# Deeptanshu-sankhwar/horizonml

Hardware: AMD Instinct MI355X
Metric: images/sec (higher is better)
Workload: dtype bf16; 1 GPU; model=resnet18_cifar10, global_batch=64, image=3x32x32, parallelism=dp1, optimizer=adam, exec=graph, comm=none

## Files before the change

### horizonml_amd/ops/csrc/bind.cpp

```cpp
#include <torch/extension.h>
#include <c10/hip/HIPStream.h>
#include <c10/hip/HIPCachingAllocator.h>

#include <memory>
#include <vector>

#include "launch.h"

namespace {

using torch::Tensor;

hipStream_t cur_stream() { return c10::hip::getCurrentHIPStream().stream(); }

bool g_deterministic = false;
void set_deterministic(bool on) {
  g_deterministic = on;
  set_kernels_deterministic(on ? 1 : 0);
}
bool deterministic_enabled() { return g_deterministic; }

void set_bn_owner(bool on) { set_kernels_bn_owner(on ? 1 : 0); }
bool bn_owner_enabled() { return kernels_bn_owner() != 0; }
std::vector<int64_t> bn_owner_launches() {
  long f = 0, b = 0;
  bn_owner_launch_counts(&f, &b);
  return {(int64_t)f, (int64_t)b};
}

bool g_dgrad_krsc = env_long("HZ_DGRAD_KRSC", 1) != 0;
void set_dgrad_krsc(bool on) { g_dgrad_krsc = on; }
bool dgrad_krsc_enabled() { return g_dgrad_krsc; }

bool g_wgrad_tr = env_long("HZ_WGRAD_TR", 1) != 0;
void set_wgrad_tr(bool on) { g_wgrad_tr = on; }
bool wgrad_tr_enabled() { return g_wgrad_tr; }

struct PendingWgrad {
  torch::Tensor x, dconv, dw;
  ConvP p;
};

bool g_wgrad_defer = false;
std::vector<PendingWgrad> g_pending;
torch::Tensor g_wgrad_ws;

void set_wgrad_defer(bool on) { g_wgrad_defer = on; }
bool wgrad_defer_enabled() { return g_wgrad_defer; }
int64_t wgrad_pending() { return (int64_t)g_pending.size(); }

static inline int cdiv_i(long a, long b) { return (int)((a + b - 1) / b); }

void flush_one_group(int lo, int hi);

void flush_wgrad() {
  if (g_pending.empty()) return;
  const int total = (int)g_pending.size();
  int lo = 0;
  while (lo < total) {
    std::vector<const void*> seen;
    int hi = lo;
    for (; hi < total; hi++) {
      const void* ptr = g_pending[hi].dw.data_ptr();
      bool dup = false;
      for (const void* q : seen)
        if (q == ptr) { dup = true; break; }
      if (dup) break;
      seen.push_back(ptr);
    }
    flush_one_group(lo, hi);
    lo = hi;
  }
  g_pending.clear();
}

void flush_wgrad_range(torch::Tensor flat, int64_t lo_elem, int64_t hi_elem) {
  if (g_pending.empty()) return;
  const char* base = (const char*)flat.data_ptr();
  const char* plo = base + lo_elem * flat.element_size();
  const char* phi = base + hi_elem * flat.element_size();
  std::vector<PendingWgrad> take, keep;
  for (auto& p : g_pending) {
    const char* q = (const char*)p.dw.data_ptr();
    if (q >= plo && q < phi)
      take.push_back(std::move(p));
    else
      keep.push_back(std::move(p));
  }
  g_pending = std::move(take);
  flush_wgrad();
  g_pending = std::move(keep);
}

void flush_one_group(int group_lo, int group_hi) {
  auto st = cur_stream();
  const int n = group_hi - group_lo;
  const PendingWgrad* pend = g_pending.data() + group_lo;
  std::vector<int> msplit(n), mchunk(n);
  std::vector<long> ws_off(n, 0);
  long ws_total = 0;
  for (int i = 0; i < n; i++) {
    const ConvP& p = pend[i].p;
    static const int mc_small = (int)env_long("HZ_WG_MCHUNK", 512);
    const int mc_base = p.M >= 32768 ? 2048 : mc_small;
    int ms = std::max(1, cdiv_i(p.M, mc_base));
    int mc = cdiv_i(cdiv_i(p.M, ms), 32) * 32;
    ms = cdiv_i(p.M, mc);
    msplit[i] = ms;
    mchunk[i] = mc;
    if (ms > 1) {
      ws_off[i] = ws_total;
      ws_total += (long)ms * p.K * p.Kd;
    }
  }
  if (ws_total > 0 &&
      (!g_wgrad_ws.defined() || g_wgrad_ws.numel() < ws_total))
    g_wgrad_ws = at::empty({ws_total},
                           pend[0].x.options().dtype(torch::kFloat32));
  float* ws_base = ws_total > 0 ? g_wgrad_ws.data_ptr<float>() : nullptr;

  auto tk3_of = [](const ConvP& p) {
    static const int kd_min = (int)env_long("HZ_WG_TK3_KD", 256);
    static const int m_min = (int)env_long("HZ_WG_TK3_M", 5000);
    return (p.Kd >= kd_min && p.M >= m_min) ? 128 : 64;
  };
  auto tko_of = [](const ConvP& p) {
    static const int k_min = (int)env_long("HZ_WG_TKO_K", 128);
    return p.K >= k_min ? 128 : 64;
  };
  for (int cls = 0; cls < 4; cls++) {
    const int tk3 = (cls & 1) ? 128 : 64;
    const int tko = (cls & 2) ? 128 : 64;
    std::vector<int> idx;
    for (int i = 0; i < n; i++)
      if (tk3_of(pend[i].p) == tk3 && tko_of(pend[i].p) == tko)
        idx.push_back(i);
    for (size_t lo = 0; lo < idx.size(); lo += WG_MAX_TASKS) {
      WgradBatchArgs a{};
      a.n = (int)std::min((size_t)WG_MAX_TASKS, idx.size() - lo);
      int blocks = 0;
      for (int j = 0; j < a.n; j++) {
        const int i = idx[lo + j];
        const PendingWgrad& pw = pend[i];
        WgradTask& t = a.t[j];
        t.X = pw.x.data_ptr();
        t.Dz = pw.dconv.data_ptr();
        t.out = msplit[i] > 1 ? ws_base + ws_off[i]
                              : pw.dw.data_ptr<float>();
        t.p = pw.p;
        t.mg = make_magic(pw.p, 1);
        t.Ntot = pw.p.K;
        t.mchunk = mchunk[i];
        t.msplit = msplit[i];
        t.tx = cdiv_i(pw.p.Kd, tk3);
        t.ty = cdiv_i(pw.p.K, tko);
        t.base = blocks;
        t.vec = (pw.p.C % 8) == 0;
        blocks += t.tx * t.ty * t.msplit;
      }
      launch_wgrad_batched_t(&a, blocks, tk3, tko, (int)g_wgrad_tr, st);
    }
  }

  WredBatchArgs r{};
  r.n = 0;
  int rblocks = 0;
  auto flush_red = [&]() {
    if (r.n > 0) launch_wgrad_reduce_batched(&r, rblocks, st);
    r.n = 0;
    rblocks = 0;
  };
  for (int i = 0; i < n; i++) {
    if (msplit[i] <= 1) continue;
    if (r.n == WG_MAX_TASKS) flush_red();
    WredTask& t = r.t[r.n++];
    t.ws = ws_base + ws_off[i];
    t.dW = pend[i].dw.data_ptr<float>();
    t.n = (long)pend[i].p.K * pend[i].p.Kd;
    t.msplit = msplit[i];
    t.base = rblocks;
    rblocks += cdiv_i(t.n, 1024);
  }
  flush_red();
}

void check_cl(const Tensor& t, const char* name) {
  TORCH_CHECK(t.is_cuda(), name, " must be on GPU");
  TORCH_CHECK(t.scalar_type() == torch::kBFloat16, name, " must be bf16");
  TORCH_CHECK(t.dim() == 4, name, " must be 4-D");
  bool cl = t.is_contiguous(at::MemoryFormat::ChannelsLast);
  bool hw1 = t.size(2) == 1 && t.size(3) == 1 && t.is_contiguous();
  TORCH_CHECK(cl || hw1, name, " must be channels_last contiguous");
}

void check_f32(const Tensor& t, const char* name) {
  TORCH_CHECK(t.is_cuda() && t.scalar_type() == torch::kFloat32 &&
                  t.is_contiguous(),
              name, " must be contiguous f32 on GPU");
}

template <class T>
T* opt_ptr(const c10::optional<Tensor>& t) {
  return t.has_value() ? t->data_ptr<T>() : nullptr;
}
void* opt_ptr(const c10::optional<Tensor>& t) {
  return t.has_value() ? t->data_ptr() : nullptr;
}

void check_probe(const c10::optional<Tensor>& prev,
                 const c10::optional<Tensor>& sumsq,
                 const c10::optional<Tensor>& out) {
  TORCH_CHECK(prev.has_value() == sumsq.has_value()
                  && prev.has_value() == out.has_value(),
              "probe tensors must be passed together");
}

Tensor empty_cl_bf16(int64_t n, int64_t c, int64_t h, int64_t w,
                     const Tensor& like) {
  return at::empty({n, c, h, w},
                   like.options().dtype(torch::kBFloat16),
                   at::MemoryFormat::ChannelsLast);
}

ConvP make_convp(const Tensor& x, int K, int R, int S, int stride, int pad) {
  ConvP p{};
  p.Nb = (int)x.size(0);
  p.C = (int)x.size(1);
  p.H = (int)x.size(2);
  p.W = (int)x.size(3);
  p.K = K;
  p.R = R;
  p.S = S;
  p.str = stride;
  p.pad = pad;
  p.Ho = (p.H + 2 * pad - R) / stride + 1;
  p.Wo = (p.W + 2 * pad - S) / stride + 1;
  p.M = p.Nb * p.Ho * p.Wo;
  p.Kd = R * S * p.C;
  return p;
}

std::vector<Tensor> conv_bn_act_fwd(
    Tensor x, Tensor w, Tensor gamma, Tensor beta, Tensor running_mean,
    Tensor running_var, int64_t stride, int64_t pad, double momentum,
    double eps, bool training, int64_t act,
    c10::optional<Tensor> residual, c10::optional<Tensor> stats_buf) {
  check_cl(x, "x");
  TORCH_CHECK(w.is_cuda() && w.scalar_type() == torch::kBFloat16 &&
                  w.is_contiguous() && w.dim() == 4,
              "w must be contiguous bf16 KRSC");
  check_f32(gamma, "gamma");
  check_f32(beta, "beta");
  int K = (int)w.size(0), R = (int)w.size(1), S = (int)w.size(2);
  TORCH_CHECK(w.size(3) == x.size(1), "w in-channels mismatch");
  ConvP p = make_convp(x, K, R, S, (int)stride, (int)pad);

  Tensor convout = empty_cl_bf16(p.Nb, K, p.Ho, p.Wo, x);
  Tensor y = empty_cl_bf16(p.Nb, K, p.Ho, p.Wo, x);
  auto fopt = x.options().dtype(torch::kFloat32);
  Tensor stats, smean, sinvstd;
  float* stats_ptr = nullptr;
  if (training) {
    smean = at::empty({K}, fopt);
    sinvstd = at::empty({K}, fopt);
  } else {
    smean = at::empty({0}, fopt);
    sinvstd = at::empty({0}, fopt);
  }
  const void* res_ptr = nullptr;
  if (residual.has_value()) {
    check_cl(*residual, "residual");
    res_ptr = residual->data_ptr();
  }
  auto st = cur_stream();
  int splitk = conv_fwd_splitk(p);
  const int own = (training && splitk > 1)
                      ? bn_owner_fwd_pick((long)p.M, K, 0) : 0;
  if (training && !own) {
    stats = stats_buf.has_value() ? *stats_buf : at::zeros({2L * K}, fopt);
    stats_ptr = stats.data_ptr<float>();
  }
  if (splitk > 1) {
    int kchunk = ((p.Kd + splitk - 1) / splitk + 31) / 32 * 32;
    splitk = (p.Kd + kchunk - 1) / kchunk;
    Tensor ws = at::empty({(long)splitk * p.M * K}, fopt);
    launch_conv_fwd_splitk(x.data_ptr(), w.data_ptr(), ws.data_ptr<float>(),
                           p, splitk, st);
    if (own) {
      launch_bn_fwd_owner(ws.data_ptr<float>(), res_ptr, y.data_ptr(),
                          convout.data_ptr(), gamma.data_ptr<float>(),
                          beta.data_ptr<float>(),
                          running_mean.data_ptr<float>(),
                          running_var.data_ptr<float>(),
                          smean.data_ptr<float>(), sinvstd.data_ptr<float>(),
                          (long)p.M, K, (float)momentum, (float)eps,
                          (int)act, splitk, own, st);
      return {y, convout, smean, sinvstd};
    }
    if (training)
      launch_stats_reduce(ws.data_ptr<float>(), stats_ptr, (long)p.M, K,
                          splitk, st);
    launch_bn_apply_f32(ws.data_ptr<float>(), res_ptr, y.data_ptr(),
                        convout.data_ptr(), stats_ptr,
                        gamma.data_ptr<float>(), beta.data_ptr<float>(),
                        running_mean.data_ptr<float>(),
                        running_var.data_ptr<float>(),
                        training ? smean.data_ptr<float>() : nullptr,
                        training ? sinvstd.data_ptr<float>() : nullptr,
                        (long)p.M, K, (float)momentum, (float)eps,
                        training ? 1 : 0, (int)act, splitk, st);
  } else {
    launch_conv_fwd(x.data_ptr(), w.data_ptr(), convout.data_ptr(),
                    g_deterministic ? nullptr : stats_ptr, p, st);
    if (g_deterministic && training)
      launch_stats_bf16_det(convout.data_ptr(), stats_ptr, (long)p.M, K,
                            st);
    launch_bn_apply(convout.data_ptr(), res_ptr, y.data_ptr(), stats_ptr,
                    gamma.data_ptr<float>(), beta.data_ptr<float>(),
                    running_mean.data_ptr<float>(),
                    running_var.data_ptr<float>(),
                    training ? smean.data_ptr<float>() : nullptr,
                    training ? sinvstd.data_ptr<float>() : nullptr,
                    (long)p.M, K, (float)momentum, (float)eps,
                    training ? 1 : 0, (int)act, st);
  }
  return {y, convout, smean, sinvstd};
}

Tensor dgrad_dx(const Tensor& dconv, const Tensor& w,
                const c10::optional<Tensor>& w_rsck, const ConvP& p,
                const c10::optional<Tensor>& dx_accum,
                const c10::optional<std::vector<Tensor>>& fuse_up,
                int up_mask_mode, hipStream_t st) {
  const bool krsc =
      !w_rsck.has_value() || w_rsck->data_ptr() == w.data_ptr();
  const Tensor& wt = krsc ? w : *w_rsck;
  TORCH_CHECK(wt.is_contiguous() && wt.scalar_type() == torch::kBFloat16,
              krsc ? "w must be contiguous bf16"
                   : "w_rsck must be contiguous bf16");
  TORCH_CHECK(wt.numel() == (int64_t)p.K * p.R * p.S * p.C,
              "dgrad weight has ", wt.numel(), " elements, expected K*R*S*C");
  auto fopt = dconv.options().dtype(torch::kFloat32);
  const int layout = krsc ? DGRAD_W_KRSC : DGRAD_W_RSCK;
  int accum = dx_accum.has_value() ? 1 : 0;
  Tensor dx = accum ? *dx_accum : empty_cl_bf16(p.Nb, p.C, p.H, p.W, dconv);
  ConvP pd = p;
  pd.M = p.Nb * p.H * p.W;
  pd.Kd = p.R * p.S * p.K;
  int splitk = conv_dgrad_splitk(p);
  const bool fuse = fuse_up.has_value();
  if (splitk > 1) {
    int kchunk = ((pd.Kd + splitk - 1) / splitk + 31) / 32 * 32;
    splitk = (pd.Kd + kchunk - 1) / kchunk;
    Tensor wsd = at::empty({(long)splitk * pd.M * p.C}, fopt);
    launch_conv_dgrad(dconv.data_ptr(), wt.data_ptr(), nullptr,
                      wsd.data_ptr<float>(), splitk, pd, 0, layout, st);
    if (fuse) {
      auto& f = *fuse_up;
      launch_cast_bnact(wsd.data_ptr<float>(), dx.data_ptr(), (long)pd.M,
                        p.C, splitk, accum, f[0].data_ptr(),
                        f[1].defined() ? f[1].data_ptr() : f[0].data_ptr(),
                        f[2].data_ptr<float>(), f[3].data_ptr<float>(),
                        f[4].data_ptr<float>(), f[5].data_ptr<float>(),
                        f[6].data_ptr<float>(), f[7].data_ptr<float>(),
                        up_mask_mode, st);
    } else {
      launch_cast_f32_bf16(wsd.data_ptr<float>(), dx.data_ptr(),
                           (long)pd.M * p.C, splitk, accum, st);
    }
  } else {
    launch_conv_dgrad(dconv.data_ptr(), wt.data_ptr(), dx.data_ptr(), nullptr,
                      1, pd, accum, layout, st);
    if (fuse) {
      auto& f = *fuse_up;
      launch_bnact_bwd_reduce(dx.data_ptr(), f[1].defined()
                                  ? f[1].data_ptr() : f[0].data_ptr(),
                              f[0].data_ptr(), f[2].data_ptr<float>(),
                              f[3].data_ptr<float>(),
                              f[4].data_ptr<float>(),
                              f[5].data_ptr<float>(),
                              f[6].data_ptr<float>(),
                              f[7].data_ptr<float>(), (long)pd.M, p.C,
                              up_mask_mode, st);
    }
  }
  return dx;
}

Tensor conv_dgrad_only(Tensor dz, Tensor w, int64_t H, int64_t W,
                       int64_t stride, int64_t pad,
                       c10::optional<Tensor> w_rsck,
                       c10::optional<Tensor> dx_accum) {
  check_cl(dz, "dz");
  TORCH_CHECK(w.dim() == 4 && w.size(0) == dz.size(1),
              "w must be [K,R,S,C] with K = dz channels");
  ConvP p{};
  p.Nb = (int)dz.size(0);
  p.C = (int)w.size(3);
  p.H = (int)H;
  p.W = (int)W;
  p.K = (int)w.size(0);
  p.R = (int)w.size(1);
  p.S = (int)w.size(2);
  p.str = (int)stride;
  p.pad = (int)pad;
  p.Ho = (p.H + 2 * p.pad - p.R) / p.str + 1;
  p.Wo = (p.W + 2 * p.pad - p.S) / p.str + 1;
  p.M = p.Nb * p.Ho * p.Wo;
  p.Kd = p.R * p.S * p.C;
  TORCH_CHECK(dz.size(2) == p.Ho && dz.size(3) == p.Wo,
              "dz spatial size does not match H, W, stride, pad");
  if (dx_accum.has_value()) {
    check_cl(*dx_accum, "dx_accum");
    TORCH_CHECK(dx_accum->size(0) == p.Nb && dx_accum->size(1) == p.C &&
                    dx_accum->size(2) == p.H && dx_accum->size(3) == p.W,
                "dx_accum must be [Nb,C,H,W]");
  }
  return dgrad_dx(dz, w, w_rsck, p, dx_accum, c10::nullopt, 0, cur_stream());
}

std::vector<Tensor> conv_bn_act_bwd(
    Tensor dy, Tensor y, Tensor x, Tensor w, c10::optional<Tensor> w_rsck,
    Tensor convout,
    Tensor gamma, Tensor beta, Tensor save_mean, Tensor save_invstd,
    int64_t stride, int64_t pad, int64_t act, bool need_dx, bool has_res,
    c10::optional<Tensor> dw_out, c10::optional<Tensor> dgamma_out,
    c10::optional<Tensor> dbeta_out, c10::optional<Tensor> dx_accum,
    c10::optional<std::vector<Tensor>> fuse_up, int64_t up_mask_mode,
    bool sums_ready, c10::optional<Tensor> sum_dz_in,
    c10::optional<Tensor> sum_dzx_in) {
  check_cl(dy, "dy");
  check_cl(y, "y");
  check_cl(x, "x");
  check_cl(convout, "convout");
  int K = (int)w.size(0), R = (int)w.size(1), S = (int)w.size(2);
  ConvP p = make_convp(x, K, R, S, (int)stride, (int)pad);
  auto fopt = x.options().dtype(torch::kFloat32);
  auto st = cur_stream();

  bool direct = dw_out.has_value();
  int mask_mode = act == 1 ? (has_res ? 1 : 2)
                 : act == 2 ? (has_res ? 3 : 4) : 0;
  Tensor sum_dz, sum_dzx;
  const int own = sums_ready ? 0 : bn_owner_bwd_pick((long)p.M, K, 0);
  if (sums_ready) {
    sum_dz = direct ? *dbeta_out : *sum_dz_in;
    sum_dzx = direct ? *dgamma_out : *sum_dzx_in;
  } else {
    sum_dz = direct ? *dbeta_out : at::zeros({K}, fopt);
    sum_dzx = direct ? *dgamma_out : at::zeros({K}, fopt);
    if (!own)
      launch_bnact_bwd_reduce(dy.data_ptr(), y.data_ptr(),
                              convout.data_ptr(),
                              save_mean.data_ptr<float>(),
                              save_invstd.data_ptr<float>(),
                              gamma.data_ptr<float>(),
                              beta.data_ptr<float>(),
                              sum_dz.data_ptr<float>(),
                              sum_dzx.data_ptr<float>(),
                              (long)p.M, K, mask_mode, st);
  }

  Tensor dconv = empty_cl_bf16(p.Nb, K, p.Ho, p.Wo, x);
  Tensor dres;
  void* dres_ptr = nullptr;
  if (has_res) {
    dres = empty_cl_bf16(p.Nb, K, p.Ho, p.Wo, x);
    dres_ptr = dres.data_ptr();
  }
  if (own)
    launch_bn_bwd_owner(dy.data_ptr(), y.data_ptr(), convout.data_ptr(),
                        save_mean.data_ptr<float>(),
                        save_invstd.data_ptr<float>(),
                        gamma.data_ptr<float>(), beta.data_ptr<float>(),
                        sum_dz.data_ptr<float>(), sum_dzx.data_ptr<float>(),
                        dconv.data_ptr(), dres_ptr, (long)p.M, K, mask_mode,
                        own, st);
  else
    launch_bn_bwd_apply(dy.data_ptr(), y.data_ptr(), convout.data_ptr(),
                        save_mean.data_ptr<float>(),
                        save_invstd.data_ptr<float>(),
                        gamma.data_ptr<float>(), beta.data_ptr<float>(),
                        sum_dz.data_ptr<float>(), sum_dzx.data_ptr<float>(),
                        dconv.data_ptr(), dres_ptr, (long)p.M, K, mask_mode,
                        st);

  Tensor dw = direct ? *dw_out
                     : at::zeros({(int64_t)K, R, S, (int64_t)p.C}, fopt);
  if (direct && g_wgrad_defer) {
    g_pending.push_back({x, dconv, dw, p});
  } else {
    int msplit = wgrad_msplit(p);
    Tensor ws;
    float* ws_ptr = nullptr;
    if (msplit > 1) {
      ws = at::empty({(long)msplit * K * p.Kd}, fopt);
      ws_ptr = ws.data_ptr<float>();
    }
    launch_wgrad(x.data_ptr(), dconv.data_ptr(), dw.data_ptr<float>(), ws_ptr,
                 p, (int)g_wgrad_tr, st);
  }

  TORCH_CHECK(need_dx || !fuse_up.has_value(),
              "fuse_up requires need_dx (the fused reduce rides the dx "
              "production)");
  Tensor dx;
  if (need_dx)
    dx = dgrad_dx(dconv, w, w_rsck, p, dx_accum, fuse_up, (int)up_mask_mode,
                  st);
  return {dx, dw, sum_dzx, sum_dz, dres};
}

void check_dw_geometry(int R, int S, int64_t stride, int H, int W,
                       int64_t pad) {
  TORCH_CHECK(R >= 1 && S >= 1 && R * S <= 25,
              "depthwise filter must have R*S <= 25 taps, got ", R, "x", S);
  TORCH_CHECK(stride >= 1, "depthwise stride must be >= 1, got ", stride);
  TORCH_CHECK(pad >= 0, "depthwise pad must be >= 0, got ", pad);
  TORCH_CHECK(H + 2 * pad >= R && W + 2 * pad >= S,
              "depthwise output must be at least 1x1: input ", H, "x", W,
              ", pad ", pad, ", filter ", R, "x", S);
}

std::vector<Tensor> dw_conv_bn_fwd(
    Tensor x, Tensor w, Tensor gamma, Tensor beta, Tensor running_mean,
    Tensor running_var, int64_t stride, int64_t pad, double momentum,
    double eps, bool training, int64_t act, c10::optional<Tensor> residual) {
  check_cl(x, "x");
  TORCH_CHECK(w.is_cuda() && w.scalar_type() == torch::kBFloat16 &&
                  w.is_contiguous() && w.dim() == 3,
              "w must be contiguous bf16 [R,S,C]");
  int Nb = (int)x.size(0), C = (int)x.size(1), H = (int)x.size(2),
      W = (int)x.size(3);
  int R = (int)w.size(0), S = (int)w.size(1);
  TORCH_CHECK((int)w.size(2) == C, "depthwise channel mismatch");
  check_dw_geometry(R, S, stride, H, W, pad);
  int Ho = (H + 2 * (int)pad - R) / (int)stride + 1;
  int Wo = (W + 2 * (int)pad - S) / (int)stride + 1;
  long M = (long)Nb * Ho * Wo;
  auto fopt = x.options().dtype(torch::kFloat32);
  Tensor convout = empty_cl_bf16(Nb, C, Ho, Wo, x);
  Tensor y = empty_cl_bf16(Nb, C, Ho, Wo, x);
  Tensor stats, smean, sinvstd;
  float* stats_ptr = nullptr;
  if (training) {
    stats = at::zeros({2L * C}, fopt);
    smean = at::empty({C}, fopt);
    sinvstd = at::empty({C}, fopt);
    stats_ptr = stats.data_ptr<float>();
  } else {
    smean = at::empty({0}, fopt);
    sinvstd = at::empty({0}, fopt);
  }
  const void* res_ptr = nullptr;
  if (residual.has_value()) {
    check_cl(*residual, "residual");
    res_ptr = residual->data_ptr();
  }
  auto st = cur_stream();
  launch_dw_fwd(x.data_ptr(), w.data_ptr(), convout.data_ptr(),
                g_deterministic ? nullptr : stats_ptr, Nb, H, W, C, Ho, Wo,
                R, S, (int)stride, (int)pad, st);
  if (g_deterministic && training)
    launch_stats_bf16_det(convout.data_ptr(), stats_ptr, M, C, st);
  launch_bn_apply(convout.data_ptr(), res_ptr, y.data_ptr(), stats_ptr,
                  gamma.data_ptr<float>(), beta.data_ptr<float>(),
                  running_mean.data_ptr<float>(),
                  running_var.data_ptr<float>(),
                  training ? smean.data_ptr<float>() : nullptr,
                  training ? sinvstd.data_ptr<float>() : nullptr, M, C,
                  (float)momentum, (float)eps, training ? 1 : 0, (int)act,
                  st);
  return {y, convout, smean, sinvstd};
}

std::vector<Tensor> dw_conv_bn_bwd(
    Tensor dy, Tensor y, Tensor x, Tensor w, Tensor convout, Tensor gamma,
    Tensor beta, Tensor save_mean, Tensor save_invstd, int64_t stride,
    int64_t pad, int64_t act, bool need_dx, bool has_res) {
  check_cl(dy, "dy");
  check_cl(x, "x");
  int Nb = (int)x.size(0), C = (int)x.size(1), H = (int)x.size(2),
      W = (int)x.size(3);
  TORCH_CHECK(w.is_cuda() && w.scalar_type() == torch::kBFloat16 &&
                  w.is_contiguous() && w.dim() == 3 && w.size(2) == C,
              "w must be contiguous bf16 [R,S,C] with C = x channels");
  int R = (int)w.size(0), S = (int)w.size(1);
  check_dw_geometry(R, S, stride, H, W, pad);
  int Ho = (int)dy.size(2), Wo = (int)dy.size(3);
  TORCH_CHECK(dy.size(0) == Nb && dy.size(1) == C &&
                  Ho == (H + 2 * (int)pad - R) / (int)stride + 1 &&
                  Wo == (W + 2 * (int)pad - S) / (int)stride + 1,
              "dy shape does not match the depthwise output of x");
  long M = (long)Nb * Ho * Wo;
  auto fopt = x.options().dtype(torch::kFloat32);
  auto st = cur_stream();
  int mask_mode = act == 1 ? (has_res ? 1 : 2)
                 : act == 2 ? (has_res ? 3 : 4) : 0;
  Tensor sum_dz = at::zeros({C}, fopt);
  Tensor sum_dzx = at::zeros({C}, fopt);
  launch_bnact_bwd_reduce(dy.data_ptr(), y.data_ptr(), convout.data_ptr(),
                          save_mean.data_ptr<float>(),
                          save_invstd.data_ptr<float>(),
                          gamma.data_ptr<float>(), beta.data_ptr<float>(),
                          sum_dz.data_ptr<float>(), sum_dzx.data_ptr<float>(),
                          M, C, mask_mode, st);
  Tensor dconv = empty_cl_bf16(Nb, C, Ho, Wo, x);
  Tensor dres;
  void* dres_ptr = nullptr;
  if (has_res) {
    dres = empty_cl_bf16(Nb, C, Ho, Wo, x);
    dres_ptr = dres.data_ptr();
  }
  launch_bn_bwd_apply(dy.data_ptr(), y.data_ptr(), convout.data_ptr(),
                      save_mean.data_ptr<float>(),
                      save_invstd.data_ptr<float>(), gamma.data_ptr<float>(),
                      beta.data_ptr<float>(), sum_dz.data_ptr<float>(),
                      sum_dzx.data_ptr<float>(), dconv.data_ptr(), dres_ptr,
                      M, C, mask_mode, st);
  Tensor dw = at::zeros({(int64_t)R, (int64_t)S, (int64_t)C}, fopt);
  launch_dw_wgrad(x.data_ptr(), dconv.data_ptr(), dw.data_ptr<float>(), Nb,
                  H, W, C, Ho, Wo, R, S, (int)stride, (int)pad, st);
  Tensor dx;
  if (need_dx) {
    dx = empty_cl_bf16(Nb, C, H, W, x);
    launch_dw_dgrad(dconv.data_ptr(), w.data_ptr(), dx.data_ptr(), Nb, H, W,
                    C, Ho, Wo, R, S, (int)stride, (int)pad, st);
  }
  return {dx, dw, sum_dzx, sum_dz, dres};
}

std::vector<Tensor> maxpool_fwd(Tensor x) {
  check_cl(x, "x");
  int Nb = (int)x.size(0), C = (int)x.size(1), H = (int)x.size(2),
      W = (int)x.size(3);
  int Hp = (H + 2 - 3) / 2 + 1, Wp = (W + 2 - 3) / 2 + 1;
  Tensor y = empty_cl_bf16(Nb, C, Hp, Wp, x);
  Tensor idx = at::empty({Nb, Hp, Wp, C}, x.options().dtype(torch::kUInt8));
  launch_maxpool_fwd(x.data_ptr(), y.data_ptr(), idx.data_ptr<unsigned char>(),
                     Nb, H, W, C, Hp, Wp, cur_stream());
  return {y, idx};
}

Tensor maxpool_bwd(Tensor dy, Tensor idx, int64_t H, int64_t W) {
  check_cl(dy, "dy");
  int Nb = (int)dy.size(0), C = (int)dy.size(1), Hp = (int)dy.size(2),
      Wp = (int)dy.size(3);
  Tensor dx = empty_cl_bf16(Nb, C, H, W, dy);
  launch_maxpool_bwd(dy.data_ptr(), idx.data_ptr<unsigned char>(),
                     dx.data_ptr(), Nb, (int)H, (int)W, C, Hp, Wp,
                     cur_stream());
  return dx;
}

Tensor avgpool_fwd(Tensor x) {
  check_cl(x, "x");
  int Nb = (int)x.size(0), C = (int)x.size(1);
  int HW = (int)(x.size(2) * x.size(3));
  Tensor y = at::empty({Nb, C}, x.options());
  launch_avgpool_fwd(x.data_ptr(), y.data_ptr(), Nb, HW, C, cur_stream());
  return y;
}

Tensor avgpool_bwd(Tensor dy, int64_t H, int64_t W) {
  TORCH_CHECK(dy.is_cuda() && dy.is_contiguous() &&
              dy.scalar_type() == torch::kBFloat16);
  int Nb = (int)dy.size(0), C = (int)dy.size(1);
  Tensor dx = empty_cl_bf16(Nb, C, H, W, dy);
  launch_avgpool_bwd(dy.data_ptr(), dx.data_ptr(), Nb, (int)(H * W), C,
                     cur_stream());
  return dx;
}

Tensor linear_fwd(Tensor x, Tensor w, c10::optional<Tensor> bias) {
  TORCH_CHECK(x.is_cuda() && x.is_contiguous() &&
              x.scalar_type() == torch::kBFloat16);
  TORCH_CHECK(w.is_cuda() && w.is_contiguous() &&
                  w.scalar_type() == torch::kBFloat16,
              "w must be contiguous bf16 on GPU");
  TORCH_CHECK(x.dim() == 2 && w.dim() == 2,
              "linear_fwd: x must be [B, In] and w [Out, In], got ", x.dim(),
              "-D x and ", w.dim(), "-D w");
  int B = (int)x.size(0), In = (int)x.size(1), Out = (int)w.size(0);
  TORCH_CHECK(w.size(1) == In, "linear_fwd: w has ", w.size(1),
              " input columns, x has ", In);
  TORCH_CHECK(In % 8 == 0, "linear_fwd: In must be a multiple of 8, got ",
              In);
  TORCH_CHECK(In <= 2048, "linear_fwd: In must be <= 2048, got ", In);
  Tensor y = at::empty({B, Out}, x.options().dtype(torch::kFloat32));
  const float* bptr = nullptr;
  if (bias.has_value()) {
    check_f32(*bias, "bias");
    TORCH_CHECK(bias->numel() == Out, "linear_fwd: bias has ", bias->numel(),
                " elements, Out is ", Out);
    bptr = bias->data_ptr<float>();
  }
  launch_linear_fwd(x.data_ptr(), w.data_ptr(), bptr, y.data_ptr<float>(), B,
                    In, Out, cur_stream());
  return y;
}

std::vector<Tensor> linear_bwd(Tensor dy, Tensor x, Tensor w, bool need_dx,
                               bool need_db, c10::optional<Tensor> dw_out,
                               c10::optional<Tensor> db_out) {
  check_f32(dy, "dy");
  TORCH_CHECK(x.is_cuda() && x.is_contiguous() &&
                  x.scalar_type() == torch::kBFloat16 && x.dim() == 2,
              "linear_bwd: x must be contiguous bf16 [B, In] on GPU");
  TORCH_CHECK(w.is_cuda() && w.is_contiguous() &&
                  w.scalar_type() == torch::kBFloat16 && w.dim() == 2,
              "linear_bwd: w must be contiguous bf16 [Out, In] on GPU");
  int B = (int)x.size(0), In = (int)x.size(1), Out = (int)w.size(0);
  TORCH_CHECK(w.size(1) == In, "linear_bwd: w has ", w.size(1),
              " input columns, x has ", In);
  TORCH_CHECK(dy.dim() == 2 && dy.size(0) == B && dy.size(1) == Out,
              "linear_bwd: dy must be [B, Out] = [", B, ", ", Out, "]");
  if (dw_out.has_value()) {
    check_f32(*dw_out, "dw_out");
    TORCH_CHECK(dw_out->dim() == 2 && dw_out->size(0) == Out &&
                    dw_out->size(1) == In,
                "linear_bwd: dw_out must be [Out, In] = [", Out, ", ", In,
                "]");
  }
  if (db_out.has_value()) {
    check_f32(*db_out, "db_out");
    TORCH_CHECK(db_out->numel() == Out, "linear_bwd: db_out has ",
                db_out->numel(), " elements, Out is ", Out);
  }
  auto fopt = x.options().dtype(torch::kFloat32);
  bool direct = dw_out.has_value();
  Tensor dx, dw = direct ? *dw_out : at::empty({Out, In}, fopt);
  Tensor db = direct ? (db_out.has_value() ? *db_out : Tensor())
                     : (need_db ? at::empty({Out}, fopt) : Tensor());
  void* dx_ptr = nullptr;
  if (need_dx) {
    dx = at::empty({B, In}, x.options());
    dx_ptr = dx.data_ptr();
  }
  launch_linear_bwd(dy.data_ptr<float>(), x.data_ptr(), w.data_ptr(), dx_ptr,
                    dw.data_ptr<float>(),
                    db.defined() ? db.data_ptr<float>() : nullptr, B, In, Out,
                    direct ? 1 : 0, cur_stream());
  return {dx, dw, db};
}

std::vector<Tensor> cross_entropy_fwd_bwd(Tensor logits, Tensor target) {
  check_f32(logits, "logits");
  TORCH_CHECK(target.scalar_type() == torch::kLong && target.is_contiguous());
  int B = (int)logits.size(0), NC = (int)logits.size(1);
  Tensor loss = at::zeros({}, logits.options());
  Tensor dlogits = at::empty({B, NC}, logits.options());
  launch_ce_fwd_bwd(logits.data_ptr<float>(), target.data_ptr<long>(),
                    loss.data_ptr<float>(), dlogits.data_ptr<float>(), B, NC,
                    cur_stream());
  return {loss, dlogits};
}

std::vector<Tensor> cross_entropy_ls_fwd_bwd(Tensor logits, Tensor target,
                                             double eps) {
  if (eps == 0.0) return cross_entropy_fwd_bwd(logits, target);
  TORCH_CHECK(eps > 0.0 && eps <= 1.0,
              "label_smoothing must be in [0, 1], got ", eps);
  check_f32(logits, "logits");
  TORCH_CHECK(target.scalar_type() == torch::kLong && target.is_contiguous());
  int B = (int)logits.size(0), NC = (int)logits.size(1);
  Tensor loss = at::zeros({}, logits.options());
  Tensor dlogits = at::empty({B, NC}, logits.options());
  launch_ce_ls_fwd_bwd(logits.data_ptr<float>(), target.data_ptr<long>(),
                       loss.data_ptr<float>(), dlogits.data_ptr<float>(), B,
                       NC, (float)eps, cur_stream());
  return {loss, dlogits};
}

Tensor gemm_bf16(Tensor a, Tensor b) {
  TORCH_CHECK(a.is_cuda() && a.is_contiguous() &&
              a.scalar_type() == torch::kBFloat16);
  TORCH_CHECK(b.is_contiguous() && b.scalar_type() == torch::kBFloat16);
  TORCH_CHECK(a.size(1) == b.size(1), "K mismatch");
  int M = (int)a.size(0), K = (int)a.size(1), N = (int)b.size(0);
  Tensor c = at::empty({M, N}, a.options());
  launch_gemm_bf16(a.data_ptr(), b.data_ptr(), c.data_ptr(), M, N, K,
                   cur_stream());
  return c;
}

Tensor wgrad_only(Tensor x, Tensor dz, int64_t K, int64_t R, int64_t S,
                  int64_t stride, int64_t pad, bool defer,
                  c10::optional<Tensor> dw_out) {
  check_cl(x, "x");
  check_cl(dz, "dz");
  ConvP p = make_convp(x, (int)K, (int)R, (int)S, (int)stride, (int)pad);
  Tensor dw = dw_out.has_value()
                  ? *dw_out
                  : at::zeros({K, R, S, (int64_t)p.C},
                              x.options().dtype(torch::kFloat32));
  if (defer) {
    g_pending.push_back({x, dz, dw, p});
  } else {
    int msplit = wgrad_msplit(p);
    Tensor ws;
    float* ws_ptr = nullptr;
    if (msplit > 1) {
      ws = at::empty({(long)msplit * p.K * p.Kd},
                     x.options().dtype(torch::kFloat32));
      ws_ptr = ws.data_ptr<float>();
    }
    launch_wgrad(x.data_ptr(), dz.data_ptr(), dw.data_ptr<float>(), ws_ptr,
                 p, (int)g_wgrad_tr, cur_stream());
  }
  return dw;
}

void adam_step(Tensor master, Tensor grad, Tensor m, Tensor v,
               c10::optional<Tensor> shadow, Tensor step_t, double lr,
               double b1, double b2, double eps, double wd, bool zero_grad,
               c10::optional<Tensor> extra_zero,
               c10::optional<Tensor> grad_bf16, double grad_scale,
               c10::optional<Tensor> probe_prev,
               c10::optional<Tensor> probe_sumsq,
               c10::optional<Tensor> probe_out) {
  check_f32(master, "master");
  check_probe(probe_prev, probe_sumsq, probe_out);
  launch_adam_step(master.data_ptr<float>(), grad.data_ptr<float>(),
                   m.data_ptr<float>(), v.data_ptr<float>(),
                   opt_ptr(shadow), step_t.data_ptr<float>(),
                   master.numel(), (float)lr, (float)b1, (float)b2,
                   (float)eps, (float)wd, zero_grad ? 1 : 0,
                   opt_ptr<float>(extra_zero),
                   extra_zero.has_value() ? extra_zero->numel() : 0,
                   opt_ptr(grad_bf16), (float)grad_scale,
                   opt_ptr<float>(probe_prev), opt_ptr<float>(probe_sumsq),
                   opt_ptr<float>(probe_out), cur_stream());
}

void sgd_step(Tensor master, Tensor grad, c10::optional<Tensor> mom,
              c10::optional<Tensor> shadow, double lr, double mu, double wd,
              bool zero_grad, c10::optional<Tensor> grad_bf16,
              double grad_scale, c10::optional<Tensor> probe_prev,
              c10::optional<Tensor> probe_sumsq,
              c10::optional<Tensor> probe_out) {
  check_f32(master, "master");
  check_probe(probe_prev, probe_sumsq, probe_out);
  launch_sgd_step(master.data_ptr<float>(), grad.data_ptr<float>(),
                  opt_ptr<float>(mom), opt_ptr(shadow), master.numel(),
                  (float)lr, (float)mu, (float)wd, zero_grad ? 1 : 0,
                  opt_ptr(grad_bf16), (float)grad_scale,
                  opt_ptr<float>(probe_prev), opt_ptr<float>(probe_sumsq),
                  opt_ptr<float>(probe_out), cur_stream());
}

const float* sched_table(const c10::optional<Tensor>& lr_table,
                         const Tensor& master, long* T) {
  *T = 0;
  if (!lr_table.has_value()) return nullptr;
  check_f32(*lr_table, "lr_table");
  TORCH_CHECK(lr_table->dim() == 1 && lr_table->numel() >= 1
                  && lr_table->device() == master.device(),
              "lr_table must be a non-empty 1-D tensor on master's device");
  *T = lr_table->numel();
  return lr_table->data_ptr<float>();
}

float* sched_scalar(const c10::optional<Tensor>& t, const Tensor& master,
                    const char* name) {
  if (!t.has_value()) return nullptr;
  check_f32(*t, name);
  TORCH_CHECK(t->numel() == 1 && t->device() == master.device(), name,
              " must hold one element on master's device");
  return t->data_ptr<float>();
}

void adam_step_sched(Tensor master, Tensor grad, Tensor m, Tensor v,
                     c10::optional<Tensor> shadow, Tensor step_t,
                     c10::optional<Tensor> lr_table,
                     c10::optional<Tensor> lr_out, double lr, double b1,
                     double b2, double eps, double wd, bool decoupled,
                     bool zero_grad, c10::optional<Tensor> extra_zero,
                     c10::optional<Tensor> grad_bf16, double grad_scale,
                     c10::optional<Tensor> probe_prev,
                     c10::optional<Tensor> probe_sumsq,
                     c10::optional<Tensor> probe_out) {
  check_f32(master, "master");
  check_probe(probe_prev, probe_sumsq, probe_out);
  TORCH_CHECK(grad.numel() == master.numel() && m.numel() == master.numel()
                  && v.numel() == master.numel(),
              "grad / m / v must match master's size");
  long T = 0;
  const float* table = sched_table(lr_table, master, &T);
  float* out = sched_scalar(lr_out, master, "lr_out");
  float* st = sched_scalar(step_t, master, "step_t");
  launch_adam_step_ex(master.data_ptr<float>(), grad.data_ptr<float>(),
                      m.data_ptr<float>(), v.data_ptr<float>(),
                      opt_ptr(shadow), st, master.numel(), (float)lr,
                      (float)b1, (float)b2, (float)eps, (float)wd,
                      zero_grad ? 1 : 0, opt_ptr<float>(extra_zero),
                      extra_zero.has_value() ? extra_zero->numel() : 0,
                      opt_ptr(grad_bf16), (float)grad_scale,
                      opt_ptr<float>(probe_prev),
                      opt_ptr<float>(probe_sumsq), opt_ptr<float>(probe_out),
                      table, T, out, decoupled ? 1 : 0, cur_stream());
}

void sgd_step_sched(Tensor master, Tensor grad, c10::optional<Tensor> mom,
                    c10::optional<Tensor> shadow,
                    c10::optional<Tensor> step_t,
                    c10::optional<Tensor> lr_table,
                    c10::optional<Tensor> lr_out, double lr, double mu,
                    double wd, bool nesterov, bool zero_grad,
                    c10::optional<Tensor> grad_bf16, double grad_scale,
                    c10::optional<Tensor> probe_prev,
                    c10::optional<Tensor> probe_sumsq,
                    c10::optional<Tensor> probe_out) {
  check_f32(master, "master");
  check_probe(probe_prev, probe_sumsq, probe_out);
  TORCH_CHECK(grad.numel() == master.numel()
                  && (!mom.has_value() || mom->numel() == master.numel()),
              "grad / mom must match master's size");
  TORCH_CHECK(!nesterov || (mom.has_value() && mu > 0.0),
              "nesterov needs a momentum buffer and momentum > 0");
  long T = 0;
  const float* table = sched_table(lr_table, master, &T);
  TORCH_CHECK(table == nullptr || step_t.has_value(),
              "lr_table needs the step_t device counter");
  float* out = sched_scalar(lr_out, master, "lr_out");
  float* st = sched_scalar(step_t, master, "step_t");
  launch_sgd_step_ex(master.data_ptr<float>(), grad.data_ptr<float>(),
                     opt_ptr<float>(mom), opt_ptr(shadow), master.numel(),
                     (float)lr, (float)mu, (float)wd, zero_grad ? 1 : 0,
                     opt_ptr(grad_bf16), (float)grad_scale,
                     opt_ptr<float>(probe_prev), opt_ptr<float>(probe_sumsq),
                     opt_ptr<float>(probe_out), st, table, T, out,
                     nesterov ? 1 : 0, cur_stream());
}

struct SegTable {
  const int* chunks;
  int nchunks;
  const float* seg_mul;
  int nseg;
};

SegTable seg_table(const Tensor& chunks, const Tensor& seg_mul,
                   const Tensor& master) {
  TORCH_CHECK(chunks.scalar_type() == torch::kInt32 && chunks.dim() == 2
                  && chunks.size(1) == 3 && chunks.size(0) >= 1
                  && chunks.is_contiguous()
                  && chunks.device() == master.device(),
              "chunks must be a contiguous int32 [nchunks,3] tensor on "
              "master's device");
  check_f32(seg_mul, "seg_mul");
  TORCH_CHECK(seg_mul.dim() == 2 && seg_mul.size(1) == 2
                  && seg_mul.size(0) >= 1 && seg_mul.is_contiguous()
                  && seg_mul.device() == master.device(),
              "seg_mul must be a contiguous f32 [nseg,2] tensor on master's "
              "device");
  return {chunks.data_ptr<int>(), (int)chunks.size(0),
          seg_mul.data_ptr<float>(), (int)seg_mul.size(0)};
}

void seg_norms(Tensor master, Tensor grad, Tensor chunks, Tensor seg_meta,
               Tensor partials, Tensor seg_norms_out, Tensor seg_mul,
               Tensor norm_out, double wd, double max_norm, bool lars,
               double eta, c10::optional<Tensor> grad_bf16,
               double grad_scale) {
  check_f32(master, "master");
  check_f32(grad, "grad");
  check_f32(partials, "partials");
  check_f32(seg_norms_out, "seg_norms");
  check_f32(norm_out, "norm_out");
  SegTable t = seg_table(chunks, seg_mul, master);
  TORCH_CHECK(grad.numel() == master.numel(), "grad must match master");
  TORCH_CHECK(seg_meta.scalar_type() == torch::kInt32
                  && seg_meta.is_contiguous() && seg_meta.dim() == 2
                  && seg_meta.size(0) == t.nseg && seg_meta.size(1) == 3
                  && seg_meta.device() == master.device(),
              "seg_meta must be a contiguous int32 [nseg,3] tensor on "
              "master's device");
  TORCH_CHECK(partials.numel() == 2L * t.nchunks
                  && seg_norms_out.numel() == 2L * t.nseg
                  && norm_out.numel() == 2 && partials.is_contiguous()
                  && seg_norms_out.is_contiguous()
                  && partials.device() == master.device()
                  && seg_norms_out.device() == master.device()
                  && norm_out.device() == master.device(),
              "partials [nchunks,2], seg_norms [nseg,2], norm_out [2] on "
              "master's device");
  TORCH_CHECK(!grad_bf16.has_value()
                  || (grad_bf16->scalar_type() == torch::kBFloat16
                      && grad_bf16->numel() == master.numel()),
              "grad_bf16 must be a bf16 tensor of master's size");
  TORCH_CHECK((uintptr_t)master.data_ptr() % 16 == 0
                  && (uintptr_t)grad.data_ptr() % 16 == 0
                  && (!grad_bf16.has_value()
                      || (uintptr_t)grad_bf16->data_ptr() % 16 == 0),
              "master / grad / grad_bf16 must be 16-byte aligned");
  launch_seg_norms(master.data_ptr<float>(), grad.data_ptr<float>(),
                   opt_ptr(grad_bf16), (float)grad_scale, t.chunks,
                   t.nchunks, seg_meta.data_ptr<int>(), t.nseg,
                   partials.data_ptr<float>(),
                   seg_norms_out.data_ptr<float>(),
                   seg_mul.data_ptr<float>(), norm_out.data_ptr<float>(),
                   (float)wd, (float)max_norm, lars ? 1 : 0, (float)eta,
                   cur_stream());
}

void adam_step_seg(Tensor master, Tensor grad, Tensor m, Tensor v,
                   c10::optional<Tensor> shadow, Tensor step_t,
                   c10::optional<Tensor> lr_table,
                   c10::optional<Tensor> lr_out, double lr, double b1,
                   double b2, double eps, bool decoupled, bool zero_grad,
                   Tensor chunks, Tensor seg_mul,
                   c10::optional<Tensor> extra_zero,
                   c10::optional<Tensor> grad_bf16, double grad_scale,
                   c10::optional<Tensor> probe_prev,
                   c10::optional<Tensor> probe_sumsq,
                   c10::optional<Tensor> probe_out) {
  check_f32(master, "master");
  check_probe(probe_prev, probe_sumsq, probe_out);
  TORCH_CHECK(grad.numel() == master.numel() && m.numel() == master.numel()
                  && v.numel() == master.numel(),
              "grad / m / v must match master's size");
  SegTable t = seg_table(chunks, seg_mul, master);
  long T = 0;
  const float* table = sched_table(lr_table, master, &T);
  float* out = sched_scalar(lr_out, master, "lr_out");
  float* st = sched_scalar(step_t, master, "step_t");
  launch_adam_step_seg(master.data_ptr<float>(), grad.data_ptr<float>(),
                       m.data_ptr<float>(), v.data_ptr<float>(),
                       opt_ptr(shadow), st, (float)lr, (float)b1, (float)b2,
                       (float)eps, zero_grad ? 1 : 0,
                       opt_ptr<float>(extra_zero),
                       extra_zero.has_value() ? extra_zero->numel() : 0,
                       opt_ptr(grad_bf16), (float)grad_scale,
                       opt_ptr<float>(probe_prev),
                       opt_ptr<float>(probe_sumsq), opt_ptr<float>(probe_out),
                       table, T, out, decoupled ? 1 : 0, t.chunks, t.nchunks,
                       t.seg_mul, cur_stream());
}

void sgd_step_seg(Tensor master, Tensor grad, c10::optional<Tensor> mom,
                  c10::optional<Tensor> shadow, c10::optional<Tensor> step_t,
                  c10::optional<Tensor> lr_table,
                  c10::optional<Tensor> lr_out, double lr, double mu,
                  bool nesterov, bool zero_grad, Tensor chunks,
                  Tensor seg_mul, c10::optional<Tensor> grad_bf16,
                  double grad_scale, c10::optional<Tensor> probe_prev,
                  c10::optional<Tensor> probe_sumsq,
                  c10::optional<Tensor> probe_out) {
  check_f32(master, "master");
  check_probe(probe_prev, probe_sumsq, probe_out);
  TORCH_CHECK(grad.numel() == master.numel()
                  && (!mom.has_value() || mom->numel() == master.numel()),
              "grad / mom must match master's size");
  TORCH_CHECK(!nesterov || (mom.has_value() && mu > 0.0),
              "nesterov needs a momentum buffer and momentum > 0");
  SegTable t = seg_table(chunks, seg_mul, master);
  long T = 0;
  const float* table = sched_table(lr_table, master, &T);
  TORCH_CHECK(table == nullptr || step_t.has_value(),
              "lr_table needs the step_t device counter");
  float* out = sched_scalar(lr_out, master, "lr_out");
  float* st = sched_scalar(step_t, master, "step_t");
  launch_sgd_step_seg(master.data_ptr<float>(), grad.data_ptr<float>(),
                      opt_ptr<float>(mom), opt_ptr(shadow), (float)lr,
                      (float)mu, zero_grad ? 1 : 0, opt_ptr(grad_bf16),
                      (float)grad_scale, opt_ptr<float>(probe_prev),
                      opt_ptr<float>(probe_sumsq), opt_ptr<float>(probe_out),
                      st, table, T, out, nesterov ? 1 : 0, t.chunks,
                      t.nchunks, t.seg_mul, cur_stream());
}

void permute_krsc_rsck(Tensor src, Tensor dst, Tensor meta,
                       int64_t max_elem) {
  TORCH_CHECK(meta.scalar_type() == torch::kInt32 && meta.is_cuda());
  launch_permute_krsc_rsck(src.data_ptr(), dst.data_ptr(),
                           meta.data_ptr<int>(), (int)meta.size(0),
                           (int)max_elem, cur_stream());
}

void grad_divergence(Tensor g, Tensor prev, Tensor sumsq, Tensor out,
                     bool skip_first) {
  launch_grad_divergence(g.data_ptr<float>(), prev.data_ptr<float>(),
                         sumsq.data_ptr<float>(), out.data_ptr<float>(),
                         g.numel(), skip_first ? 1 : 0, cur_stream());
}

void bn_reduce_bench(Tensor dy, Tensor y, Tensor x, Tensor mean,
                     Tensor invstd, Tensor gamma, Tensor beta, Tensor sdz,
                     Tensor sdzx, int64_t M, int64_t C, int64_t mask) {
  launch_bnact_bwd_reduce(dy.data_ptr(), y.data_ptr(), x.data_ptr(),
                          mean.data_ptr<float>(), invstd.data_ptr<float>(),
                          gamma.data_ptr<float>(), beta.data_ptr<float>(),
                          sdz.data_ptr<float>(), sdzx.data_ptr<float>(), M,
                          (int)C, (int)mask, cur_stream());
}

int64_t bn_fwd_pair_bench(Tensor ws, c10::optional<Tensor> res, Tensor y,
                          Tensor convout, Tensor stats, Tensor gamma,
                          Tensor beta, Tensor rmean, Tensor rvar,
                          Tensor smean, Tensor sinvstd, int64_t M, int64_t C,
                          int64_t nsplit, int64_t act, int64_t lpr) {
  TORCH_CHECK(ws.numel() >= nsplit * M * C && y.numel() >= M * C &&
                  convout.numel() >= M * C && stats.numel() >= 2 * C,
              "bn_fwd_pair_bench: buffers smaller than nsplit*M*C");
  const void* rp = opt_ptr(res);
  auto st = cur_stream();
  if (lpr == 0) {
    launch_stats_reduce(ws.data_ptr<float>(), stats.data_ptr<float>(), M,
                        (int)C, (int)nsplit, st);
    launch_bn_apply_f32(ws.data_ptr<float>(), rp, y.data_ptr(),
                        convout.data_ptr(), stats.data_ptr<float>(),
                        gamma.data_ptr<float>(), beta.data_ptr<float>(),
                        rmean.data_ptr<float>(), rvar.data_ptr<float>(),
                        smean.data_ptr<float>(), sinvstd.data_ptr<float>(),
                        M, (int)C, 0.1f, 1e-5f, 1, (int)act, (int)nsplit,
                        st);
    return 0;
  }
  int own = bn_owner_fwd_pick(M, (int)C, (int)lpr);
  TORCH_CHECK(own > 0, "owner forward kernel does not take M=", M, " C=", C);
  launch_bn_fwd_owner(ws.data_ptr<float>(), rp, y.data_ptr(),
                      convout.data_ptr(), gamma.data_ptr<float>(),
                      beta.data_ptr<float>(), rmean.data_ptr<float>(),
                      rvar.data_ptr<float>(), smean.data_ptr<float>(),
                      sinvstd.data_ptr<float>(), M, (int)C, 0.1f, 1e-5f,
                      (int)act, (int)nsplit, own, st);
  return own;
}

int64_t bn_bwd_pair_bench(Tensor dy, Tensor y, Tensor x, Tensor mean,
                          Tensor invstd, Tensor gamma, Tensor beta,
                          Tensor sdz, Tensor sdzx, Tensor dconv,
                          c10::optional<Tensor> dres, int64_t M, int64_t C,
                          int64_t mask, int64_t lpr) {
  TORCH_CHECK(dy.numel() >= M * C && y.numel() >= M * C &&
                  x.numel() >= M * C && dconv.numel() >= M * C &&
                  sdz.numel() >= C && sdzx.numel() >= C,
              "bn_bwd_pair_bench: buffers smaller than M*C");
  void* drp = opt_ptr(dres);
  auto st = cur_stream();
  if (lpr == 0) {
    launch_bnact_bwd_reduce(dy.data_ptr(), y.data_ptr(), x.data_ptr(),
                            mean.data_ptr<float>(), invstd.data_ptr<float>(),
                            gamma.data_ptr<float>(), beta.data_ptr<float>(),
                            sdz.data_ptr<float>(), sdzx.data_ptr<float>(), M,
                            (int)C, (int)mask, st);
    launch_bn_bwd_apply(dy.data_ptr(), y.data_ptr(), x.data_ptr(),
                        mean.data_ptr<float>(), invstd.data_ptr<float>(),
                        gamma.data_ptr<float>(), beta.data_ptr<float>(),
                        sdz.data_ptr<float>(), sdzx.data_ptr<float>(),
                        dconv.data_ptr(), drp, M, (int)C, (int)mask, st);
    return 0;
  }
  int own = bn_owner_bwd_pick(M, (int)C, (int)lpr);
  TORCH_CHECK(own > 0, "owner backward kernel does not take M=", M, " C=", C);
  launch_bn_bwd_owner(dy.data_ptr(), y.data_ptr(), x.data_ptr(),
                      mean.data_ptr<float>(), invstd.data_ptr<float>(),
                      gamma.data_ptr<float>(), beta.data_ptr<float>(),
                      sdz.data_ptr<float>(), sdzx.data_ptr<float>(),
                      dconv.data_ptr(), drp, M, (int)C, (int)mask, own, st);
  return own;
}

Tensor normalize_u8(Tensor x, double mean, double std) {
  TORCH_CHECK(x.dim() == 4 && x.dtype() == torch::kUInt8 && x.is_cuda()
                  && x.is_contiguous(),
              "normalize_u8 expects contiguous NCHW uint8 on GPU");
  const long N = x.size(0), C = x.size(1), H = x.size(2), W = x.size(3);
  auto y = at::empty({N, C, H, W},
                     x.options().dtype(torch::kBFloat16),
                     at::MemoryFormat::ChannelsLast);
  launch_normalize_u8(x.data_ptr(), y.data_ptr(), N * C * H * W, (int)C,
                      H * W, (float)mean, (float)std, cur_stream());
  return y;
}

Tensor augment_normalize_u8(Tensor x, Tensor state, double mean, double std,
                            int64_t pad, bool flip,
                            c10::optional<Tensor> params) {
  TORCH_CHECK(x.dim() == 4 && x.dtype() == torch::kUInt8 && x.is_cuda()
                  && x.is_contiguous(),
              "augment_normalize_u8 expects contiguous NCHW uint8 on GPU");
  TORCH_CHECK(pad >= 0 && pad <= 127,
              "augment_normalize_u8: pad must be in [0, 127], got ", pad);
  TORCH_CHECK(state.is_cuda() && state.dtype() == torch::kInt64
                  && state.is_contiguous() && state.numel() >= 2
                  && state.device() == x.device(),
              "augment_normalize_u8: state must be a contiguous int64 GPU "
              "tensor with >= 2 elements (key, step)");
  const long N = x.size(0), C = x.size(1), H = x.size(2), W = x.size(3);
  TORCH_CHECK(N * C * H * W < (1L << 31),
              "augment_normalize_u8: batch too large for 32-bit indexing");
  const int* pp = nullptr;
  if (params.has_value()) {
    const Tensor& p = *params;
    TORCH_CHECK(p.is_cuda() && p.dtype() == torch::kInt32
                    && p.is_contiguous() && p.numel() == N
                    && p.device() == x.device(),
                "augment_normalize_u8: params must be a contiguous int32 GPU "
                "tensor with N = ", N, " elements");
    pp = p.data_ptr<int>();
  }
  auto y = at::empty({N, C, H, W},
                     x.options().dtype(torch::kBFloat16),
                     at::MemoryFormat::ChannelsLast);
  launch_augment_normalize_u8(x.data_ptr(), y.data_ptr(), state.data_ptr(),
                              pp, N, (int)C, (int)H, (int)W, (int)pad,
                              flip ? 1 : 0, (float)mean, (float)std,
                              cur_stream());
  return y;
}

}

PYBIND11_MODULE(TORCH_EXTENSION_NAME, m) {
  m.def("conv_bn_act_fwd", &conv_bn_act_fwd);
  m.def("conv_bn_act_bwd", &conv_bn_act_bwd);
  m.def("dw_conv_bn_fwd", &dw_conv_bn_fwd);
  m.def("dw_conv_bn_bwd", &dw_conv_bn_bwd);
  m.def("maxpool_fwd", &maxpool_fwd);
  m.def("maxpool_bwd", &maxpool_bwd);
  m.def("avgpool_fwd", &avgpool_fwd);
  m.def("avgpool_bwd", &avgpool_bwd);
  m.def("linear_fwd", &linear_fwd);
  m.def("linear_bwd", &linear_bwd);
  m.def("cross_entropy_fwd_bwd", &cross_entropy_fwd_bwd);
  m.def("gemm_bf16", &gemm_bf16);
  m.def("adam_step", &adam_step);
  m.def("sgd_step", &sgd_step);
  m.def("cross_entropy_ls_fwd_bwd", &cross_entropy_ls_fwd_bwd);
  m.def("adam_step_sched", &adam_step_sched, py::arg("master"),
        py::arg("grad"), py::arg("m"), py::arg("v"), py::arg("shadow"),
        py::arg("step_t"), py::arg("lr_table"), py::arg("lr_out"),
        py::arg("lr"), py::arg("b1"), py::arg("b2"), py::arg("eps"),
        py::arg("wd"), py::arg("decoupled"), py::arg("zero_grad"),
        py::arg("extra_zero") = py::none(), py::arg("grad_bf16") = py::none(),
        py::arg("grad_scale") = 1.0, py::arg("probe_prev") = py::none(),
        py::arg("probe_sumsq") = py::none(),
        py::arg("probe_out") = py::none());
  m.def("sgd_step_sched", &sgd_step_sched, py::arg("master"),
        py::arg("grad"), py::arg("mom"), py::arg("shadow"), py::arg("step_t"),
        py::arg("lr_table"), py::arg("lr_out"), py::arg("lr"), py::arg("mu"),
        py::arg("wd"), py::arg("nesterov"), py::arg("zero_grad"),
        py::arg("grad_bf16") = py::none(), py::arg("grad_scale") = 1.0,
        py::arg("probe_prev") = py::none(),
        py::arg("probe_sumsq") = py::none(),
        py::arg("probe_out") = py::none());
  m.def("seg_norms", &seg_norms, py::arg("master"), py::arg("grad"),
        py::arg("chunks"), py::arg("seg_meta"), py::arg("partials"),
        py::arg("seg_norms"), py::arg("seg_mul"), py::arg("norm_out"),
        py::arg("wd"), py::arg("max_norm"), py::arg("lars"), py::arg("eta"),
        py::arg("grad_bf16") = py::none(), py::arg("grad_scale") = 1.0);
  m.def("adam_step_seg", &adam_step_seg, py::arg("master"), py::arg("grad"),
        py::arg("m"), py::arg("v"), py::arg("shadow"), py::arg("step_t"),
        py::arg("lr_table"), py::arg("lr_out"), py::arg("lr"), py::arg("b1"),
        py::arg("b2"), py::arg("eps"), py::arg("decoupled"),
        py::arg("zero_grad"), py::arg("chunks"), py::arg("seg_mul"),
        py::arg("extra_zero") = py::none(), py::arg("grad_bf16") = py::none(),
        py::arg("grad_scale") = 1.0, py::arg("probe_prev") = py::none(),
        py::arg("probe_sumsq") = py::none(),
        py::arg("probe_out") = py::none());
  m.def("sgd_step_seg", &sgd_step_seg, py::arg("master"), py::arg("grad"),
        py::arg("mom"), py::arg("shadow"), py::arg("step_t"),
        py::arg("lr_table"), py::arg("lr_out"), py::arg("lr"), py::arg("mu"),
        py::arg("nesterov"), py::arg("zero_grad"), py::arg("chunks"),
        py::arg("seg_mul"), py::arg("grad_bf16") = py::none(),
        py::arg("grad_scale") = 1.0, py::arg("probe_prev") = py::none(),
        py::arg("probe_sumsq") = py::none(),
        py::arg("probe_out") = py::none());
  m.def("permute_krsc_rsck", &permute_krsc_rsck);
  m.def("grad_divergence", &grad_divergence);
  m.def("normalize_u8", &normalize_u8);
  m.def("augment_normalize_u8", &augment_normalize_u8, py::arg("x"),
        py::arg("state"), py::arg("mean"), py::arg("std"), py::arg("pad"),
        py::arg("flip"), py::arg("params") = py::none());
  m.def("bn_reduce_bench", &bn_reduce_bench);
  m.def("bn_fwd_pair_bench", &bn_fwd_pair_bench);
  m.def("bn_bwd_pair_bench", &bn_bwd_pair_bench);
  m.def("set_bn_owner", &set_bn_owner);
  m.def("bn_owner_enabled", &bn_owner_enabled);
  m.def("bn_owner_launches", &bn_owner_launches);
  m.def("set_deterministic", &set_deterministic);
  m.def("deterministic_enabled", &deterministic_enabled);
  m.def("set_wgrad_defer", &set_wgrad_defer);
  m.def("wgrad_defer_enabled", &wgrad_defer_enabled);
  m.def("wgrad_pending", &wgrad_pending);
  m.def("flush_wgrad", &flush_wgrad);
  m.def("flush_wgrad_range", &flush_wgrad_range);
  m.def("wgrad_only", &wgrad_only);
  m.def("conv_dgrad_only", &conv_dgrad_only);
  m.def("set_dgrad_krsc", &set_dgrad_krsc);
  m.def("dgrad_krsc_enabled", &dgrad_krsc_enabled);
  m.def("set_wgrad_tr", &set_wgrad_tr);
  m.def("wgrad_tr_enabled", &wgrad_tr_enabled);
}
```

### horizonml_amd/ops/csrc/conv_kernels.hip

```cpp
#include "common.h"

template <int MODE>
DEV int a_addr(const ConvP& p, const MagicP& mg, int m, int k, bool& valid) {
  if (MODE == 0) {
    valid = (m < p.M) & (k < p.Kd);
    return m * p.Kd + k;
  } else if (MODE == 1) {
    unsigned n = fdiv(m, mg, 0), hw = fmod(m, n, mg, 0);
    unsigned ho = fdiv(hw, mg, 1), wo = fmod(hw, ho, mg, 1);
    unsigned r = fdiv(k, mg, 2), rm = fmod(k, r, mg, 2);
    unsigned sx = fdiv(rm, mg, 3), c = fmod(rm, sx, mg, 3);
    int hi = (int)ho * p.str - p.pad + (int)r;
    int wi = (int)wo * p.str - p.pad + (int)sx;
    valid = (m < p.M) & (k < p.Kd) & (hi >= 0) & (hi < p.H) & (wi >= 0) & (wi < p.W);
    return (((int)n * p.H + hi) * p.W + wi) * p.C + (int)c;
  } else {
    unsigned n = fdiv(m, mg, 0), hw = fmod(m, n, mg, 0);
    unsigned hi = fdiv(hw, mg, 1), wi = fmod(hw, hi, mg, 1);
    unsigned r = fdiv(k, mg, 2), rm = fmod(k, r, mg, 2);
    unsigned sx = fdiv(rm, mg, 3), ko = fmod(rm, sx, mg, 3);
    int hs = (int)hi + p.pad - (int)r, ws = (int)wi + p.pad - (int)sx;
    bool ok = (m < p.M) & (k < p.Kd) & (hs >= 0) & (ws >= 0) &&
              (hs % p.str == 0) && (ws % p.str == 0);
    int ho = hs / p.str, wo = ws / p.str;
    ok = ok && (ho < p.Ho) && (wo < p.Wo);
    valid = ok;
    return (((int)n * p.Ho + ho) * p.Wo + wo) * p.K + (int)ko;
  }
}

template <int MODE>
DEV int b_addr(const ConvP& p, const MagicP& mg, int n, int k, int Ntot,
               bool& valid) {
  if (MODE == 2) {
    unsigned rs = fdiv(k, mg, 3), ko = fmod(k, rs, mg, 3);
    valid = (n < Ntot) & (k < p.Kd);
    return ((int)rs * p.C + n) * p.K + (int)ko;
  }
  valid = (n < Ntot) & (k < p.Kd);
  return n * p.Kd + k;
}

template <int MODE, bool VEC>
DEV V8 load8_a(const bf16* __restrict__ src, const ConvP& p,
               const MagicP& mg, int m, int k) {
  V8 v;
  if (VEC) {
    bool ok;
    int a = a_addr<MODE>(p, mg, m, k, ok);
    if (ok) v.u = *(const uint4*)(src + a);
    else v.u = uint4{0, 0, 0, 0};
  } else if (MODE == 1) {
    int n = m / (p.Ho * p.Wo), hw = m % (p.Ho * p.Wo);
    int ho = hw / p.Wo, wo = hw % p.Wo;
    int r = k / (p.S * p.C), rm = k % (p.S * p.C);
    int s = rm / p.C, c = rm % p.C;
    int hi = ho * p.str - p.pad + r, wi = wo * p.str - p.pad + s;
    const bool mok = m < p.M;
    int kk = k;
#pragma unroll
    for (int e = 0; e < 8; e++) {
      bool ok = mok && kk < p.Kd && hi >= 0 && hi < p.H && wi >= 0 &&
                wi < p.W;
      v.e[e] = ok ? src[((n * p.H + hi) * p.W + wi) * p.C + c] : (bf16)0.f;
      kk++;
      if (++c == p.C) {
        c = 0;
        ++wi;
        if (++s == p.S) {
          s = 0;
          wi -= p.S;
          ++r;
          ++hi;
        }
      }
    }
  } else {
    for (int e = 0; e < 8; e++) {
      bool ok;
      int a = a_addr<MODE>(p, mg, m, k + e, ok);
      v.e[e] = ok ? src[a] : (bf16)0.f;
    }
  }
  return v;
}

template <int MODE, bool VEC>
DEV V8 load8_b(const bf16* __restrict__ src, const ConvP& p,
               const MagicP& mg, int n, int k, int Ntot) {
  V8 v;
  if (VEC) {
    bool ok;
    int a = b_addr<MODE>(p, mg, n, k, Ntot, ok);
    if (ok) v.u = *(const uint4*)(src + a);
    else v.u = uint4{0, 0, 0, 0};
  } else {
    for (int e = 0; e < 8; e++) {
      bool ok;
      int a = b_addr<MODE>(p, mg, n, k + e, Ntot, ok);
      v.e[e] = ok ? src[a] : (bf16)0.f;
    }
  }
  return v;
}

template <int TN>
DEV int lds_tr_off(int k, int n) {
  const int f = TN == 64 ? (((k >> 1) & 1) | (((k >> 3) & 1) << 1))
                         : ((k & 3) | (((k >> 3) & 1) << 2));
  return k * TN + ((((n >> 4) ^ f)) << 4) + (n & 15);
}

template <bool VEC>
DEV V8 load8_b_krsc(const bf16* __restrict__ src, const ConvP& p,
                    const MagicP& mg, int n, int k, int kend, int Ntot) {
  V8 v;
  unsigned rs = fdiv(k, mg, 3), ko = fmod(k, rs, mg, 3);
  const bool kok = k < kend;
  const int a = ((int)ko * p.R * p.S + (int)rs) * p.C + n;
  if (VEC) {
    if (kok && n < Ntot) v.u = *(const uint4*)(src + a);
    else v.u = uint4{0, 0, 0, 0};
  } else {
    for (int e = 0; e < 8; e++)
      v.e[e] = (kok && n + e < Ntot) ? src[a + e] : (bf16)0.f;
  }
  return v;
}

typedef __attribute__((ext_vector_type(4))) __bf16 bf16x4;
typedef __attribute__((address_space(3))) bf16x4 lds_bf16x4;

DEV bf16x4 lds_read_tr16(const bf16* sp) {
  return __builtin_amdgcn_ds_read_tr16_b64_v4bf16((lds_bf16x4*)sp);
}

#define LDA 40

template <int MODE, bool VECA, bool VECB, bool STATS, bool SPLIT,
          int TM = 64, int TN = 64, bool KRSC = false>
__global__ __launch_bounds__(256) void k_conv_mfma(
    const bf16* __restrict__ A, const bf16* __restrict__ Bw,
    bf16* __restrict__ Y, float* __restrict__ ws_out,
    float* __restrict__ stats, ConvP p, MagicP mg, int Ntot, int kchunk,
    int accum) {
  constexpr int AC = TM / 64;
  constexpr int BC = TN / 64;
  constexpr int MI = TM / 32;
  constexpr int NI = TN / 32;
  constexpr int WM = TM / 2, WN = TN / 2;
  static_assert(!KRSC || MODE == 2, "KRSC is a dgrad B layout");
  static_assert(!KRSC || TN == 64 || TN == 128,
                "lds_tr_off covers TN 64/128");
  __shared__ __attribute__((aligned(16))) bf16 As[2][TM * LDA];
  __shared__ __attribute__((aligned(16))) bf16 Bs[2][TN * LDA];

  const int m0 = blockIdx.y * TM, n0 = blockIdx.x * TN;
  const int kbeg = SPLIT ? blockIdx.z * kchunk : 0;
  const int kend = SPLIT ? min(p.Kd, kbeg + kchunk) : p.Kd;
  const int tid = threadIdx.x;
  const int srow = tid >> 2, scol = (tid & 3) * 8;
  const int lane = tid & 63, wave = tid >> 6;
  const int wr = wave >> 1, wc = wave & 1;
  const int fr = lane & 15, fk = lane >> 4;
  const int bkrow = tid / (TN / 8), bncol = (tid % (TN / 8)) * 8;
  constexpr int BKSTEP = 256 / (TN / 8);

  auto load_b = [&](int j, int kt) -> V8 {
    if (KRSC)
      return load8_b_krsc<VECB>(Bw, p, mg, n0 + bncol,
                                kt + j * BKSTEP + bkrow, kend, Ntot);
    return load8_b<MODE, VECB>(Bw, p, mg, n0 + j * 64 + srow, kt + scol,
                               Ntot);
  };
  auto store_b = [&](int b, int j, const V8& v) {
    if (KRSC)
      *(V8*)&Bs[b][lds_tr_off<TN>(j * BKSTEP + bkrow, bncol)] = v;
    else
      *(V8*)&Bs[b][(j * 64 + srow) * LDA + scol] = v;
  };
  int boff[NI];
#pragma unroll
  for (int ni = 0; ni < NI; ni++)
    boff[ni] = lds_tr_off<TN>(fk * 8 + (fr >> 2),
                            wc * WN + ni * 16 + (fr & 3) * 4);

  f32x4 acc[MI][NI] = {};

#pragma unroll
  for (int j = 0; j < AC; j++) {
    V8 a0 = load8_a<MODE, VECA>(A, p, mg, m0 + j * 64 + srow, kbeg + scol);
    *(V8*)&As[0][(j * 64 + srow) * LDA + scol] = a0;
  }
#pragma unroll
  for (int j = 0; j < BC; j++) store_b(0, j, load_b(j, kbeg));
  V8 a_nx[AC], b_nx[BC];
  if (kbeg + 32 < kend) {
#pragma unroll
    for (int j = 0; j < AC; j++)
      a_nx[j] = load8_a<MODE, VECA>(A, p, mg, m0 + j * 64 + srow,
                                    kbeg + 32 + scol);
#pragma unroll
    for (int j = 0; j < BC; j++) b_nx[j] = load_b(j, kbeg + 32);
  }
  __syncthreads();

  int buf = 0;
  for (int k0 = kbeg; k0 < kend; k0 += 32) {
    if (k0 + 32 < kend) {
#pragma unroll
      for (int j = 0; j < AC; j++)
        *(V8*)&As[buf ^ 1][(j * 64 + srow) * LDA + scol] = a_nx[j];
#pragma unroll
      for (int j = 0; j < BC; j++) store_b(buf ^ 1, j, b_nx[j]);
      if (k0 + 64 < kend) {
#pragma unroll
        for (int j = 0; j < AC; j++)
          a_nx[j] = load8_a<MODE, VECA>(A, p, mg, m0 + j * 64 + srow,
                                        k0 + 64 + scol);
#pragma unroll
        for (int j = 0; j < BC; j++) b_nx[j] = load_b(j, k0 + 64);
      }
    }
    bf16x8 af[MI], bf[NI];
#pragma unroll
    for (int mi = 0; mi < MI; mi++)
      af[mi] =
          *(const bf16x8*)&As[buf][(wr * WM + mi * 16 + fr) * LDA + fk * 8];
#pragma unroll
    for (int ni = 0; ni < NI; ni++) {
      if (KRSC) {
        bf16x4 lo = lds_read_tr16(&Bs[buf][boff[ni]]);
        bf16x4 hi = lds_read_tr16(&Bs[buf][boff[ni] + 4 * TN]);
        bf[ni] = __builtin_shufflevector(lo, hi, 0, 1, 2, 3, 4, 5, 6, 7);
      } else {
        bf[ni] =
            *(const bf16x8*)&Bs[buf][(wc * WN + ni * 16 + fr) * LDA + fk * 8];
      }
    }
#pragma unroll
    for (int mi = 0; mi < MI; mi++)
#pragma unroll
      for (int ni = 0; ni < NI; ni++)
        acc[mi][ni] = __builtin_amdgcn_mfma_f32_16x16x32_bf16(
            af[mi], bf[ni], acc[mi][ni], 0, 0, 0);
    buf ^= 1;
    __syncthreads();
  }

  float ssum[NI], ssq[NI];
#pragma unroll
  for (int ni = 0; ni < NI; ni++) ssum[ni] = ssq[ni] = 0.f;
#pragma unroll
  for (int mi = 0; mi < MI; mi++) {
#pragma unroll
    for (int ni = 0; ni < NI; ni++) {
      int gn = n0 + wc * WN + ni * 16 + fr;
#pragma unroll
      for (int q = 0; q < 4; q++) {
        int gm = m0 + wr * WM + mi * 16 + fk * 4 + q;
        if (gm < p.M && gn < Ntot) {
          float v = acc[mi][ni][q];
          if (SPLIT) {
            ws_out[(long)blockIdx.z * p.M * Ntot + (long)gm * Ntot + gn] = v;
          } else {
            long yi = (long)gm * Ntot + gn;
            if (accum) v += b2f(Y[yi]);
            Y[yi] = f2b(v);
            if (STATS) {
              ssum[ni] += v;
              ssq[ni] += v * v;
            }
          }
        }
      }
    }
  }
  if (STATS && !SPLIT && stats != nullptr) {
#pragma unroll
    for (int ni = 0; ni < NI; ni++) {
      float s = ssum[ni] + __shfl_xor(ssum[ni], 16, 64);
      s += __shfl_xor(s, 32, 64);
      float s2 = ssq[ni] + __shfl_xor(ssq[ni], 16, 64);
      s2 += __shfl_xor(s2, 32, 64);
      int gn = n0 + wc * WN + ni * 16 + fr;
      if (fk == 0 && gn < Ntot) {
        atomicAdd(&stats[gn], s);
        atomicAdd(&stats[Ntot + gn], s2);
      }
    }
  }
}

#define LDW 40

template <int TK3, int TKO = 64>
union WgradSmemT {
  struct {
    bf16 At[TK3 * LDW];
    bf16 Dt[TKO * LDW];
  } s;
  struct {
    __attribute__((aligned(16))) bf16 A[32 * TK3];
    __attribute__((aligned(16))) bf16 D[32 * TKO];
  } r;
  float out[64][TK3 == 64 ? 65 : 131];
};
using WgradSmem = WgradSmemT<64, 64>;

template <bool VECA, int TK3, int TKO>
DEV void wgrad_mloop_tr(const bf16* __restrict__ X,
                        const bf16* __restrict__ Dz, const ConvP& p,
                        const MagicP& mg, int Ntot, int k3_0, int n0,
                        int mbeg, int mend, WgradSmemT<TK3, TKO>& smem,
                        f32x4 (&acc)[TK3 / 32][TKO / 32]) {
  constexpr int AC = TK3 / 64, DC = TKO / 64;
  constexpr int MI = TK3 / 32, NI = TKO / 32;
  const int tid = threadIdx.x;
  const int sm = tid >> 3, sv = (tid & 7) * 8;
  const int lane = tid & 63, wave = tid >> 6;
  const int wr = wave >> 1, wc = wave & 1;
  const int fr = lane & 15, fk = lane >> 4;

  V8 a_nx[AC], d_nx[DC];
  auto load_tile = [&](int mt) {
#pragma unroll
    for (int j = 0; j < AC; j++)
      a_nx[j] = load8_a<1, VECA>(X, p, mg, mt + sm, k3_0 + j * 64 + sv);
#pragma unroll
    for (int j = 0; j < DC; j++) {
      int m = mt + sm, n = n0 + j * 64 + sv;
      if (m < p.M && n < Ntot)
        d_nx[j].u = *(const uint4*)(Dz + (long)m * Ntot + n);
      else
        d_nx[j].u = uint4{0, 0, 0, 0};
    }
  };
  bf16* At = smem.r.A;
  bf16* Dt = smem.r.D;
  int aoff[MI], doff[NI];
#pragma unroll
  for (int mi = 0; mi < MI; mi++)
    aoff[mi] = lds_tr_off<TK3>(fk * 8 + (fr >> 2),
                               wr * (TK3 / 2) + mi * 16 + (fr & 3) * 4);
#pragma unroll
  for (int ni = 0; ni < NI; ni++)
    doff[ni] = lds_tr_off<TKO>(fk * 8 + (fr >> 2),
                               wc * (TKO / 2) + ni * 16 + (fr & 3) * 4);

  load_tile(mbeg);
  for (int m0 = mbeg; m0 < mend; m0 += 32) {
#pragma unroll
    for (int j = 0; j < AC; j++)
      *(V8*)&At[lds_tr_off<TK3>(sm, j * 64 + sv)] = a_nx[j];
#pragma unroll
    for (int j = 0; j < DC; j++)
      *(V8*)&Dt[lds_tr_off<TKO>(sm, j * 64 + sv)] = d_nx[j];
    __syncthreads();
    if (m0 + 32 < mend) load_tile(m0 + 32);
    bf16x8 af[MI], bf[NI];
#pragma unroll
    for (int mi = 0; mi < MI; mi++) {
      bf16x4 lo = lds_read_tr16(&At[aoff[mi]]);
      bf16x4 hi = lds_read_tr16(&At[aoff[mi] + 4 * TK3]);
      af[mi] = __builtin_shufflevector(lo, hi, 0, 1, 2, 3, 4, 5, 6, 7);
    }
#pragma unroll
    for (int ni = 0; ni < NI; ni++) {
      bf16x4 lo = lds_read_tr16(&Dt[doff[ni]]);
      bf16x4 hi = lds_read_tr16(&Dt[doff[ni] + 4 * TKO]);
      bf[ni] = __builtin_shufflevector(lo, hi, 0, 1, 2, 3, 4, 5, 6, 7);
    }
#pragma unroll
    for (int mi = 0; mi < MI; mi++)
#pragma unroll
      for (int ni = 0; ni < NI; ni++)
        acc[mi][ni] = __builtin_amdgcn_mfma_f32_16x16x32_bf16(
            af[mi], bf[ni], acc[mi][ni], 0, 0, 0);
    __syncthreads();
  }
}

template <bool VECA, int TK3 = 64, int TKO = 64, bool TR = false>
DEV void wgrad_tile(const bf16* __restrict__ X, const bf16* __restrict__ Dz,
                    float* __restrict__ out, const ConvP& p,
                    const MagicP& mg, int Ntot, int mchunk, int tx, int ty,
                    int z, bool split, WgradSmemT<TK3, TKO>& smem) {
  constexpr int AC = TK3 / 64;
  constexpr int DC = TKO / 64;
  constexpr int MI = TK3 / 32;
  constexpr int NI = TKO / 32;
  bf16* At = smem.s.At;
  bf16* Dt = smem.s.Dt;
  const int k3_0 = tx * TK3, n0 = ty * TKO;
  const int mbeg = z * mchunk;
  const int mend = min(p.M, mbeg + mchunk);
  const int tid = threadIdx.x;
  const int sm = tid >> 3, sv = (tid & 7) * 8;
  const int lane = tid & 63, wave = tid >> 6;
  const int wr = wave >> 1, wc = wave & 1;
  const int fr = lane & 15, fk = lane >> 4;

  f32x4 acc[MI][NI] = {};

  if (TR) {
    wgrad_mloop_tr<VECA, TK3, TKO>(X, Dz, p, mg, Ntot, k3_0, n0, mbeg, mend,
                                   smem, acc);
  } else {
  V8 a_nx[AC], d_nx[DC];
#pragma unroll
  for (int j = 0; j < AC; j++)
    a_nx[j] = load8_a<1, VECA>(X, p, mg, mbeg + sm, k3_0 + j * 64 + sv);
#pragma unroll
  for (int j = 0; j < DC; j++) {
    int m = mbeg + sm, n = n0 + j * 64 + sv;
    if (m < p.M && n < Ntot)
      d_nx[j].u = *(const uint4*)(Dz + (long)m * Ntot + n);
    else
      d_nx[j].u = uint4{0, 0, 0, 0};
  }
  const int smlo = sm & 7, smhi = sm >> 3;
  for (int m0 = mbeg; m0 < mend; m0 += 32) {
#pragma unroll
    for (int j = 0; j < AC; j++)
#pragma unroll
      for (int e = 0; e < 8; e++) {
        int row = j * 64 + sv + e;
        int smx = smlo | (((smhi ^ row) & 3) << 3);
        At[row * LDW + smx] = a_nx[j].e[e];
      }
#pragma unroll
    for (int j = 0; j < DC; j++)
#pragma unroll
      for (int e = 0; e < 8; e++) {
        int row = j * 64 + sv + e;
        int smx = smlo | (((smhi ^ row) & 3) << 3);
        Dt[row * LDW + smx] = d_nx[j].e[e];
      }
    __syncthreads();
    if (m0 + 32 < mend) {
#pragma unroll
      for (int j = 0; j < AC; j++)
        a_nx[j] = load8_a<1, VECA>(X, p, mg, m0 + 32 + sm,
                                   k3_0 + j * 64 + sv);
#pragma unroll
      for (int j = 0; j < DC; j++) {
        int m = m0 + 32 + sm, n = n0 + j * 64 + sv;
        if (m < p.M && n < Ntot)
          d_nx[j].u = *(const uint4*)(Dz + (long)m * Ntot + n);
        else
          d_nx[j].u = uint4{0, 0, 0, 0};
      }
    }
    bf16x8 af[MI], bf[NI];
#pragma unroll
    for (int mi = 0; mi < MI; mi++) {
      int row = wr * (TK3 / 2) + mi * 16 + fr;
      af[mi] = *(const bf16x8*)&At[row * LDW + ((fk ^ row) & 3) * 8];
    }
#pragma unroll
    for (int ni = 0; ni < NI; ni++) {
      int row = wc * (TKO / 2) + ni * 16 + fr;
      bf[ni] = *(const bf16x8*)&Dt[row * LDW + ((fk ^ row) & 3) * 8];
    }
#pragma unroll
    for (int mi = 0; mi < MI; mi++)
#pragma unroll
      for (int ni = 0; ni < NI; ni++)
        acc[mi][ni] = __builtin_amdgcn_mfma_f32_16x16x32_bf16(
            af[mi], bf[ni], acc[mi][ni], 0, 0, 0);
    __syncthreads();
  }
  }
  float* dst = out + (split ? (long)z * Ntot * (long)p.Kd : 0L);
  constexpr int CCH = TK3 / 4;
  const int ko_r = tid >> 2, cch = (tid & 3) * CCH;
#pragma unroll
  for (int pass = 0; pass < TKO / 64; pass++) {
    __syncthreads();
    if (TKO == 64 || wc == pass) {
#pragma unroll
      for (int mi = 0; mi < MI; mi++)
#pragma unroll
        for (int ni = 0; ni < NI; ni++) {
          int ko_l = wc * (TKO / 2) + ni * 16 + fr - pass * 64;
#pragma unroll
          for (int q = 0; q < 4; q++)
            smem.out[ko_l][wr * (TK3 / 2) + mi * 16 + fk * 4 + q] =
                acc[mi][ni][q];
        }
    }
    __syncthreads();
    const int gko = n0 + pass * 64 + ko_r;
    if (gko < Ntot) {
      long base = (long)gko * p.Kd + k3_0 + cch;
      if (k3_0 + cch + CCH <= p.Kd) {
#pragma unroll
        for (int e = 0; e < CCH; e += 4) {
          float4 v = *(const float4*)&smem.out[ko_r][cch + e];
          if (!split) {
            float4 d = *(const float4*)&dst[base + e];
            v.x += d.x; v.y += d.y; v.z += d.z; v.w += d.w;
          }
          *(float4*)&dst[base + e] = v;
        }
      } else {
        for (int e = 0; e < CCH && k3_0 + cch + e < p.Kd; e++)
          dst[base + e] =
              smem.out[ko_r][cch + e] + (split ? 0.f : dst[base + e]);
      }
    }
  }
}

template <bool VECA, bool TR>
__global__ __launch_bounds__(256) void k_wgrad(
    const bf16* __restrict__ X, const bf16* __restrict__ Dz,
    float* __restrict__ dW, ConvP p, MagicP mg, int Ntot, int mchunk) {
  __shared__ WgradSmem smem;
  wgrad_tile<VECA, 64, 64, TR>(X, Dz, dW, p, mg, Ntot, mchunk, blockIdx.x,
                               blockIdx.y, blockIdx.z, gridDim.z > 1, smem);
}

__global__ __launch_bounds__(256) void k_wgrad_reduce(
    const float* __restrict__ ws, float* __restrict__ dW, long n,
    int msplit) {
  long i4 = ((long)blockIdx.x * blockDim.x + threadIdx.x) * 4;
  long stride = (long)gridDim.x * blockDim.x * 4;
  for (; i4 + 4 <= n; i4 += stride) {
    float4 v = *(const float4*)&ws[i4];
    for (int z = 1; z < msplit; z++) {
      float4 w = *(const float4*)&ws[(long)z * n + i4];
      v.x += w.x; v.y += w.y; v.z += w.z; v.w += w.w;
    }
    float4 d = *(float4*)&dW[i4];
    d.x += v.x; d.y += v.y; d.z += v.z; d.w += v.w;
    *(float4*)&dW[i4] = d;
  }
  if (blockIdx.x == 0 && threadIdx.x < 4) {
    long tail = n & ~3L;
    for (long i = tail + threadIdx.x; i < n; i += 4) {
      float v = ws[i];
      for (int z = 1; z < msplit; z++) v += ws[(long)z * n + i];
      dW[i] += v;
    }
  }
}

template <int TK3, int TKO, bool TR>
__global__ __launch_bounds__(256) void k_wgrad_batched(WgradBatchArgs a) {
  int bid = blockIdx.x;
  int i = 0;
  while (i + 1 < a.n && bid >= a.t[i + 1].base) i++;
  const WgradTask& t = a.t[i];
  int local = bid - t.base;
  int nt = t.tx * t.ty;
  int z = local / nt, rem = local - z * nt;
  int ty = rem / t.tx, tx = rem - ty * t.tx;
  __shared__ WgradSmemT<TK3, TKO> smem;
  const bf16* X = (const bf16*)t.X;
  const bf16* Dz = (const bf16*)t.Dz;
  if (t.vec)
    wgrad_tile<true, TK3, TKO, TR>(X, Dz, t.out, t.p, t.mg, t.Ntot, t.mchunk,
                                   tx, ty, z, t.msplit > 1, smem);
  else
    wgrad_tile<false, TK3, TKO, TR>(X, Dz, t.out, t.p, t.mg, t.Ntot, t.mchunk,
                                    tx, ty, z, t.msplit > 1, smem);
}

__global__ __launch_bounds__(256) void k_wgrad_reduce_batched(
    WredBatchArgs a) {
  int bid = blockIdx.x;
  int i = 0;
  while (i + 1 < a.n && bid >= a.t[i + 1].base) i++;
  const WredTask& t = a.t[i];
  long i4 = ((long)(bid - t.base) * 256 + threadIdx.x) * 4;
  if (i4 + 4 <= t.n) {
    float4 v = *(const float4*)&t.ws[i4];
    for (int z = 1; z < t.msplit; z++) {
      float4 w = *(const float4*)&t.ws[(long)z * t.n + i4];
      v.x += w.x; v.y += w.y; v.z += w.z; v.w += w.w;
    }
    float4 d = *(float4*)&t.dW[i4];
    d.x += v.x; d.y += v.y; d.z += v.z; d.w += v.w;
    *(float4*)&t.dW[i4] = d;
  } else {
    for (long j = i4; j < t.n; j++) {
      float v = t.ws[j];
      for (int z = 1; z < t.msplit; z++) v += t.ws[(long)z * t.n + j];
      t.dW[j] += v;
    }
  }
}

static inline int cdiv_h(int a, int b) { return (a + b - 1) / b; }

static inline int pick_splitk(int tiles, int Kd) {
  static const int tile_min = (int)env_long("HZ_SK_TILES", 256);
  static const int kd_min = (int)env_long("HZ_SK_KD", 1024);
  if (tiles >= tile_min || Kd < kd_min) return 1;
  int sk = cdiv_h(256, tiles);
  int maxsk = cdiv_h(Kd, 32);
  if (sk > maxsk) sk = maxsk;
  if (sk > 32) sk = 32;
  return sk;
}

static inline int pick_tile(int M, int N);
static inline int pick_tile_dgrad(int M, int N);

static int sk_fill(int dgrad) {
  static const int vf = (int)env_long("HZ_SK_FILL", 0);
  static const int vd = (int)env_long("HZ_SK_FILL_DG", 256);
  return dgrad ? vd : vf;
}

static int fill_splitk(int blocks128, int Kd, int fillmin) {
  int sk = cdiv_h(fillmin, blocks128);
  int maxsk = cdiv_h(Kd, 32);
  if (sk > maxsk) sk = maxsk;
  if (sk > 8) sk = 8;
  return sk;
}

extern "C" int conv_fwd_splitk(ConvP p) {
  int tiles = cdiv_h(p.K, 64) * cdiv_h(p.M, 64);
  int sk = pick_splitk(tiles, p.Kd);
  if (sk == 1 && sk_fill(0) > 0 && p.Kd >= 512
      && pick_tile(p.M, p.K) == 2) {
    int blocks = cdiv_h(p.M, 128) * cdiv_h(p.K, 128);
    if (blocks < sk_fill(0)) return fill_splitk(blocks, p.Kd, sk_fill(0));
  }
  return sk;
}

extern "C" int conv_dgrad_splitk(ConvP p) {
  static const int kd_min_dg = (int)env_long("HZ_SK_KD_DG", 512);
  static const int tile_min_dg = (int)env_long("HZ_SK_TILES_DG", 256);
  int tiles = cdiv_h(p.C, 64) * cdiv_h(p.Nb * p.H * p.W, 64);
  int Kd = p.R * p.S * p.K;
  if (tiles >= tile_min_dg || Kd < kd_min_dg) {
    int M = p.Nb * p.H * p.W;
    if (sk_fill(1) > 0 && Kd >= 512 && pick_tile_dgrad(M, p.C) == 2) {
      int blocks = cdiv_h(M, 128) * cdiv_h(p.C, 128);
      if (blocks < sk_fill(1)) return fill_splitk(blocks, Kd, sk_fill(1));
    }
    return 1;
  }
  int sk = cdiv_h(256, tiles);
  int maxsk = cdiv_h(Kd, 32);
  if (sk > maxsk) sk = maxsk;
  if (sk > 32) sk = 32;
  return sk;
}

#define STEM_WPITCH 232
template <bool STATS>
__global__ __launch_bounds__(256) void k_stem_conv(
    const bf16* __restrict__ X, const bf16* __restrict__ Wk,
    bf16* __restrict__ Y, float* __restrict__ stats, ConvP p, int rows_pb,
    int wo_pad, int xpitch, int bpi) {
  extern __shared__ bf16 sm[];
  bf16* Wl = sm;
  bf16* Xl = sm + 64 * STEM_WPITCH;
  const int tid = threadIdx.x;
  const int lane = tid & 63, wave = tid >> 6;
  const int wr = wave >> 1, wc = wave & 1;
  const int fr = lane & 15, fk = lane >> 4;

  for (int i = tid; i < 64 * STEM_WPITCH; i += 256) {
    int ch = i / STEM_WPITCH, col = i - ch * STEM_WPITCH;
    int r = col >> 5, j = col & 31;
    bf16 v = (bf16)0.f;
    if (ch < p.K && r < 7 && j < 21 && col < 7 * 32)
      v = Wk[ch * 147 + r * 21 + j];
    Wl[i] = v;
  }

  const int n = blockIdx.x / bpi;
  const int ho0 = (blockIdx.x - n * bpi) * rows_pb;
  const int nrows = rows_pb * 2 + 5;
  const int hi0 = ho0 * 2 - 3;
  const int rowlen = p.W * 3;
  for (int i = tid; i < nrows * xpitch; i += 256) {
    int rr = i / xpitch, col = i - rr * xpitch;
    int hi = hi0 + rr;
    bf16 v = (bf16)0.f;
    int e = col - 9;
    if (hi >= 0 && hi < p.H && e >= 0 && e < rowlen)
      v = X[((long)(n * p.H + hi) * p.W) * 3 + e];
    Xl[i] = v;
  }
  __syncthreads();

  f32x4 acc[4][2] = {};
  int abase[4];
#pragma unroll
  for (int mi = 0; mi < 4; mi++) {
    int ml = wr * 64 + mi * 16 + fr;
    int hl = ml / wo_pad;
    int wo = ml - hl * wo_pad;
    if (hl >= rows_pb) hl = rows_pb - 1;
    abase[mi] = hl * 2 * xpitch + wo * 6 + fk * 8;
  }
#pragma unroll
  for (int r = 0; r < 7; r++) {
    bf16x8 af[4], bf[2];
#pragma unroll
    for (int mi = 0; mi < 4; mi++) {
      const uint32_t* xu = (const uint32_t*)&Xl[abase[mi] + r * xpitch];
      union { uint32_t u[4]; bf16x8 v; } a;
      a.u[0] = xu[0];
      a.u[1] = xu[1];
      a.u[2] = xu[2];
      a.u[3] = xu[3];
      af[mi] = a.v;
    }
#pragma unroll
    for (int ni = 0; ni < 2; ni++) {
      int ch = wc * 32 + ni * 16 + fr;
      bf[ni] = *(const bf16x8*)&Wl[ch * STEM_WPITCH + r * 32 + fk * 8];
    }
#pragma unroll
    for (int mi = 0; mi < 4; mi++)
#pragma unroll
      for (int ni = 0; ni < 2; ni++)
        acc[mi][ni] = __builtin_amdgcn_mfma_f32_16x16x32_bf16(
            af[mi], bf[ni], acc[mi][ni], 0, 0, 0);
  }

  float ssum[2] = {0.f, 0.f}, ssq[2] = {0.f, 0.f};
#pragma unroll
  for (int mi = 0; mi < 4; mi++) {
#pragma unroll
    for (int ni = 0; ni < 2; ni++) {
      int gn = wc * 32 + ni * 16 + fr;
#pragma unroll
      for (int q = 0; q < 4; q++) {
        int ml = wr * 64 + mi * 16 + fk * 4 + q;
        int hl = ml / wo_pad;
        int wo = ml - hl * wo_pad;
        if (hl < rows_pb && ho0 + hl < p.Ho && wo < p.Wo && gn < p.K) {
          float v = acc[mi][ni][q];
          long gm = (long)(n * p.Ho + ho0 + hl) * p.Wo + wo;
          Y[gm * p.K + gn] = f2b(v);
          if (STATS) {
            ssum[ni] += v;
            ssq[ni] += v * v;
          }
        }
      }
    }
  }
  if (STATS && stats != nullptr) {
#pragma unroll
    for (int ni = 0; ni < 2; ni++) {
      float s = ssum[ni] + __shfl_xor(ssum[ni], 16, 64);
      s += __shfl_xor(s, 32, 64);
      float s2 = ssq[ni] + __shfl_xor(ssq[ni], 16, 64);
      s2 += __shfl_xor(s2, 32, 64);
      int gn = wc * 32 + ni * 16 + fr;
      if (fk == 0 && gn < p.K) {
        atomicAdd(&stats[gn], s);
        atomicAdd(&stats[p.K + gn], s2);
      }
    }
  }
}

static inline bool stem_eligible(const ConvP& p) {
  static const int on = (int)env_long("HZ_STEM_DIRECT", 0);
  return on && p.C == 3 && p.R == 7 && p.S == 7 && p.str == 2 &&
         p.pad == 3 && p.K <= 64 && p.Wo <= 128;
}

static void launch_stem_conv(const bf16* x, const bf16* w, bf16* y,
                             float* stats, const ConvP& p, hipStream_t st) {
  int wo_pad = ((p.Wo + 15) / 16) * 16;
  int rows_pb = 128 / wo_pad;
  if (rows_pb < 1) rows_pb = 1;
  int bpi = (p.Ho + rows_pb - 1) / rows_pb;
  int amax = 6 * (wo_pad - 1) + 33;
  int xp = 9 + 3 * p.W + 8;
  if (xp < amax) xp = amax;
  xp = ((xp + 7) / 8) * 8;
  int nrows = rows_pb * 2 + 5;
  size_t lds = (size_t)(64 * STEM_WPITCH + nrows * xp) * sizeof(bf16);
  dim3 grid(p.Nb * bpi);
  if (stats != nullptr)
    k_stem_conv<true><<<grid, 256, lds, st>>>(x, w, y, stats, p, rows_pb,
                                              wo_pad, xp, bpi);
  else
    k_stem_conv<false><<<grid, 256, lds, st>>>(x, w, y, nullptr, p, rows_pb,
                                               wo_pad, xp, bpi);
}

static inline int pick_tile_env(int M, int N, int fill, int m_min,
                                int m_min256) {
  if (M < m_min) return 0;
  if (M >= m_min256 && N < 128
      && (long)cdiv_h(M, 256) * cdiv_h(N, 64) >= fill)
    return 3;
  if (N >= 128 && (long)cdiv_h(M, 128) * cdiv_h(N, 128) >= fill) return 2;
  if ((long)cdiv_h(M, 128) * cdiv_h(N, 64) >= fill) return 1;
  return 0;
}

static inline int pick_tile_dgrad(int M, int N) {
  static const int fill = (int)env_long("HZ_TILE_FILL_DG", 192);
  static const int m_min = (int)env_long("HZ_TILE_M_MIN_DG", 16384);
  static const int m256 = (int)env_long("HZ_TILE_M256_DG", 65536);
  return pick_tile_env(M, N, fill, m_min, m256);
}

static inline int pick_tile(int M, int N) {
  static const int fill = (int)env_long("HZ_TILE_FILL", 192);
  static const int m_min = (int)env_long("HZ_TILE_M_MIN", 16384);
  static const int m_min256 = (int)env_long("HZ_TILE_M256", 65536);
  return pick_tile_env(M, N, fill, m_min, m_min256);
}

extern "C" void launch_conv_fwd(const void* x, const void* w, void* y,
                                float* stats, ConvP p, hipStream_t st) {
  if (stem_eligible(p)) {
    launch_stem_conv((const bf16*)x, (const bf16*)w, (bf16*)y, stats, p,
                     st);
    return;
  }
  bool vec = (p.C % 8) == 0 && (p.Kd % 8) == 0;
  bool s = stats != nullptr;
  auto A = (const bf16*)x;
  auto B = (const bf16*)w;
  auto Y = (bf16*)y;
  MagicP mg = make_magic(p, 1);
  int tile = pick_tile(p.M, p.K);
#define CASE_T(VA, VB, ST, TM, TN)                                     \
  k_conv_mfma<1, VA, VB, ST, false, TM, TN><<<grid, 256, 0, st>>>(     \
      A, B, Y, nullptr, stats, p, mg, p.K, 0, 0)
#define DISPATCH(TM, TN)                                               \
  do {                                                                 \
    dim3 grid(cdiv_h(p.K, TN), cdiv_h(p.M, TM));                       \
    if (vec && s) CASE_T(true, true, true, TM, TN);                    \
    else if (vec) CASE_T(true, true, false, TM, TN);                   \
    else if (s) CASE_T(false, false, true, TM, TN);                    \
    else CASE_T(false, false, false, TM, TN);                          \
  } while (0)
  if (tile == 3) DISPATCH(256, 64);
  else if (tile == 2) DISPATCH(128, 128);
  else if (tile == 1) DISPATCH(128, 64);
  else DISPATCH(64, 64);
#undef DISPATCH
#undef CASE_T
}

extern "C" void launch_conv_fwd_splitk(const void* x, const void* w,
                                       float* ws, ConvP p, int splitk,
                                       hipStream_t st) {
  int kchunk = cdiv_h(cdiv_h(p.Kd, splitk), 32) * 32;
  splitk = cdiv_h(p.Kd, kchunk);
  bool vec = (p.C % 8) == 0 && (p.Kd % 8) == 0;
  auto A = (const bf16*)x;
  auto B = (const bf16*)w;
  MagicP mg = make_magic(p, 1);
  int tile = pick_tile(p.M, p.K);
#define SK_T(VA, VB, TM, TN)                                              k_conv_mfma<1, VA, VB, false, true, TM, TN><<<grid, 256, 0, st>>>(          A, B, nullptr, ws, nullptr, p, mg, p.K, kchunk, 0)
#define DISPATCH(TM, TN)                                                  do {                                                                      dim3 grid(cdiv_h(p.K, TN), cdiv_h(p.M, TM), splitk);                    if (vec) SK_T(true, true, TM, TN);                                      else SK_T(false, false, TM, TN);                                      } while (0)
  if (tile == 3) DISPATCH(256, 64);
  else if (tile == 2) DISPATCH(128, 128);
  else if (tile == 1) DISPATCH(128, 64);
  else DISPATCH(64, 64);
#undef DISPATCH
#undef SK_T
}

template <int TM, int TN>
static void dgrad_krsc_t(const bf16* A, const bf16* B, bf16* dx, float* ws,
                         bool split, int splitk, int kchunk, const ConvP& p,
                         const MagicP& mg, int accum, hipStream_t st) {
  dim3 grid(cdiv_h(p.C, TN), cdiv_h(p.M, TM), split ? splitk : 1);
  const bool va = (p.K % 8) == 0, vb = (p.C % 8) == 0;
#define KRSC_T(VA, VB)                                                      \
  do {                                                                      \
    if (split)                                                              \
      k_conv_mfma<2, VA, VB, false, true, TM, TN, true>                     \
          <<<grid, 256, 0, st>>>(A, B, nullptr, ws, nullptr, p, mg, p.C,    \
                                 kchunk, 0);                                \
    else                                                                    \
      k_conv_mfma<2, VA, VB, false, false, TM, TN, true>                    \
          <<<grid, 256, 0, st>>>(A, B, dx, nullptr, nullptr, p, mg, p.C, 0, \
                                 accum);                                    \
  } while (0)
  if (va && vb) KRSC_T(true, true);
  else if (va) KRSC_T(true, false);
  else if (vb) KRSC_T(false, true);
  else KRSC_T(false, false);
#undef KRSC_T
}

extern "C" void launch_conv_dgrad(const void* dz, const void* w, void* dx,
                                  float* ws, int splitk, ConvP p, int accum,
                                  int w_layout, hipStream_t st) {
  bool vec = (p.K % 8) == 0;
  auto A = (const bf16*)dz;
  auto B = (const bf16*)w;
  if (w_layout == DGRAD_W_KRSC) {
    const bool split = splitk > 1;
    int kchunk = 0;
    if (split) {
      kchunk = cdiv_h(cdiv_h(p.Kd, splitk), 32) * 32;
      splitk = cdiv_h(p.Kd, kchunk);
    }
    MagicP mg = make_magic(p, 2);
    int tile = pick_tile_dgrad(p.M, p.C);
#define DISPATCH(TM, TN)                                                  \
  dgrad_krsc_t<TM, TN>(A, B, (bf16*)dx, ws, split, splitk, kchunk, p, mg, \
                       accum, st)
    if (tile == 3) DISPATCH(256, 64);
    else if (tile == 2) DISPATCH(128, 128);
    else if (tile == 1) DISPATCH(128, 64);
    else DISPATCH(64, 64);
#undef DISPATCH
    return;
  }
  if (splitk > 1) {
    int kchunk = cdiv_h(cdiv_h(p.Kd, splitk), 32) * 32;
    splitk = cdiv_h(p.Kd, kchunk);
    MagicP mg = make_magic(p, 2);
    int tile = pick_tile_dgrad(p.M, p.C);
#define SKD_T(VA, VB, TM, TN)                                             k_conv_mfma<2, VA, VB, false, true, TM, TN><<<grid, 256, 0, st>>>(          A, B, nullptr, ws, nullptr, p, mg, p.C, kchunk, 0)
#define DISPATCH(TM, TN)                                                  do {                                                                      dim3 grid(cdiv_h(p.C, TN), cdiv_h(p.M, TM), splitk);                    if (vec) SKD_T(true, true, TM, TN);                                     else SKD_T(false, false, TM, TN);                                     } while (0)
    if (tile == 3) DISPATCH(256, 64);
    else if (tile == 2) DISPATCH(128, 128);
    else if (tile == 1) DISPATCH(128, 64);
    else DISPATCH(64, 64);
#undef DISPATCH
#undef SKD_T
  } else {
    MagicP mg = make_magic(p, 2);
    int tile = pick_tile_dgrad(p.M, p.C);
#define DGRAD_T(VA, VB, TM, TN)                                         \
  k_conv_mfma<2, VA, VB, false, false, TM, TN><<<grid, 256, 0, st>>>(   \
      A, B, (bf16*)dx, nullptr, nullptr, p, mg, p.C, 0, accum)
#define DISPATCH(TM, TN)                                                \
  do {                                                                  \
    dim3 grid(cdiv_h(p.C, TN), cdiv_h(p.M, TM));                        \
    if (vec) DGRAD_T(true, true, TM, TN);                               \
    else DGRAD_T(false, false, TM, TN);                                 \
  } while (0)
    if (tile == 3) DISPATCH(256, 64);
    else if (tile == 2) DISPATCH(128, 128);
    else if (tile == 1) DISPATCH(128, 64);
    else DISPATCH(64, 64);
#undef DISPATCH
#undef DGRAD_T
  }
}

extern "C" void launch_gemm_bf16(const void* a, const void* b, void* c, int M,
                                 int N, int K, hipStream_t st) {
  ConvP p{};
  p.M = M;
  p.Kd = K;
  dim3 grid(cdiv_h(N, 64), cdiv_h(M, 64));
  bool vec = (K % 8) == 0;
  MagicP mg{};
  if (vec)
    k_conv_mfma<0, true, true, false, false>
        <<<grid, 256, 0, st>>>((const bf16*)a, (const bf16*)b, (bf16*)c,
                               nullptr, nullptr, p, mg, N, 0, 0);
  else
    k_conv_mfma<0, false, false, false, false>
        <<<grid, 256, 0, st>>>((const bf16*)a, (const bf16*)b, (bf16*)c,
                               nullptr, nullptr, p, mg, N, 0, 0);
}

template <bool TR>
static void wgrad_batched_tr(const WgradBatchArgs& a, int blocks, int tk3,
                             int tko, hipStream_t st) {
  if (tk3 == 128 && tko == 128)
    k_wgrad_batched<128, 128, TR><<<blocks, 256, 0, st>>>(a);
  else if (tk3 == 128)
    k_wgrad_batched<128, 64, TR><<<blocks, 256, 0, st>>>(a);
  else if (tko == 128)
    k_wgrad_batched<64, 128, TR><<<blocks, 256, 0, st>>>(a);
  else
    k_wgrad_batched<64, 64, TR><<<blocks, 256, 0, st>>>(a);
}

extern "C" void launch_wgrad_batched_t(const WgradBatchArgs* args, int blocks,
                                       int tk3, int tko, int tr,
                                       hipStream_t st) {
  if (blocks <= 0) return;
  if (tr) wgrad_batched_tr<true>(*args, blocks, tk3, tko, st);
  else wgrad_batched_tr<false>(*args, blocks, tk3, tko, st);
}

extern "C" void launch_wgrad_reduce_batched(const WredBatchArgs* args,
                                            int blocks, hipStream_t st) {
  if (blocks > 0) k_wgrad_reduce_batched<<<blocks, 256, 0, st>>>(*args);
}

extern "C" int wgrad_msplit(ConvP p) {
  int tiles = cdiv_h(p.Kd, 64) * cdiv_h(p.K, 64);
  int msplit = max(1, min(cdiv_h(p.M, 32), 512 / max(1, tiles)));
  int mchunk = cdiv_h(cdiv_h(p.M, msplit), 32) * 32;
  return cdiv_h(p.M, mchunk);
}

extern "C" void launch_wgrad(const void* x, const void* dz, float* dw,
                             float* ws, ConvP p, int tr, hipStream_t st) {
  int msplit = wgrad_msplit(p);
  int mchunk = cdiv_h(cdiv_h(p.M, msplit), 32) * 32;
  dim3 grid(cdiv_h(p.Kd, 64), cdiv_h(p.K, 64), msplit);
  bool vec = (p.C % 8) == 0;
  float* out = msplit > 1 ? ws : dw;
  MagicP mg = make_magic(p, 1);
#define WGRAD_T(VA, TR)                                               \
  k_wgrad<VA, TR><<<grid, 256, 0, st>>>((const bf16*)x, (const bf16*)dz, \
                                        out, p, mg, p.K, mchunk)
#define DISPATCH(TR)            \
  do {                          \
    if (vec) WGRAD_T(true, TR); \
    else WGRAD_T(false, TR);    \
  } while (0)
  if (tr) DISPATCH(true);
  else DISPATCH(false);
#undef DISPATCH
#undef WGRAD_T
  if (msplit > 1) {
    long n = (long)p.K * p.Kd;
    int blocks = (int)min((n / 4 + 255) / 256, (long)1024);
    k_wgrad_reduce<<<blocks, 256, 0, st>>>(ws, dw, n, msplit);
  }
}
```

### horizonml_amd/ops/csrc/launch.h

```cpp
#pragma once
#include <hip/hip_runtime_api.h>

#include <cstdlib>
#include <type_traits>

struct ConvP {
  int Nb, H, W, C, K;
  int Ho, Wo, R, S;
  int str, pad;
  int M, Kd;
};

struct MagicP {
  unsigned m[4];
  int s[4];
  unsigned d[4];
};

constexpr int WG_MAX_TASKS = 20;

struct WgradTask {
  const void* X;
  const void* Dz;
  float* out;
  ConvP p;
  MagicP mg;
  int Ntot, mchunk, msplit, tx, ty;
  int base;
  int vec;
};

struct WgradBatchArgs {
  int n;
  WgradTask t[WG_MAX_TASKS];
};

struct WredTask {
  const float* ws;
  float* dW;
  long n;
  int msplit;
  int base;
};

struct WredBatchArgs {
  int n;
  WredTask t[WG_MAX_TASKS];
};

static_assert(sizeof(WgradBatchArgs) <= 4096 && sizeof(WredBatchArgs) <= 4096,
              "batched wgrad task tables must fit the kernarg segment");
static_assert(std::is_trivially_copyable_v<WgradBatchArgs> &&
                  std::is_trivially_copyable_v<WredBatchArgs>,
              "batched wgrad task tables are copied into the kernarg segment");

enum DgradWLayout { DGRAD_W_RSCK = 0, DGRAD_W_KRSC = 1 };

inline void magic_u32(unsigned d, unsigned* m, int* sh) {
  if (d <= 1) { *m = 0; *sh = 0; return; }
  int p = 0;
  while ((1ull << p) < d) p++;
  *m = (unsigned)((((unsigned long long)((1ull << p) - d) << 32) / d) + 1);
  *sh = p;
}

inline MagicP make_magic(const ConvP& p, int mode) {
  MagicP mg{};
  unsigned d[4];
  if (mode == 2) {
    d[0] = (unsigned)(p.H * p.W);
    d[1] = (unsigned)p.W;
    d[2] = (unsigned)(p.S * p.K);
    d[3] = (unsigned)p.K;
  } else {
    d[0] = (unsigned)(p.Ho * p.Wo);
    d[1] = (unsigned)p.Wo;
    d[2] = (unsigned)(p.S * p.C);
    d[3] = (unsigned)p.C;
  }
  for (int i = 0; i < 4; i++) {
    mg.d[i] = d[i] ? d[i] : 1;
    magic_u32(mg.d[i], &mg.m[i], &mg.s[i]);
  }
  return mg;
}

inline long env_long(const char* name, long dflt) {
  const char* e = getenv(name);
  return e ? atol(e) : dflt;
}

extern "C" {

int conv_fwd_splitk(ConvP p);
int conv_dgrad_splitk(ConvP p);
void launch_conv_fwd(const void* x, const void* w, void* y, float* stats,
                     ConvP p, hipStream_t st);
void launch_conv_fwd_splitk(const void* x, const void* w, float* ws, ConvP p,
                            int splitk, hipStream_t st);
void launch_conv_dgrad(const void* dz, const void* w, void* dx, float* ws,
                       int splitk, ConvP p, int accum, int w_layout,
                       hipStream_t st);
void launch_gemm_bf16(const void* a, const void* b, void* c, int M, int N,
                      int K, hipStream_t st);
int wgrad_msplit(ConvP p);
void launch_wgrad(const void* x, const void* dz, float* dw, float* ws,
                  ConvP p, int tr, hipStream_t st);
void launch_wgrad_batched_t(const WgradBatchArgs* args, int blocks, int tk3,
                            int tko, int tr, hipStream_t st);
void launch_wgrad_reduce_batched(const WredBatchArgs* args, int blocks,
                                 hipStream_t st);

void set_kernels_deterministic(int on);
void set_kernels_bn_owner(int on);
int kernels_bn_owner();
void bn_owner_launch_counts(long* fwd, long* bwd);
int bn_owner_fwd_pick(long M, int C, int lpr_req);
int bn_owner_bwd_pick(long M, int C, int lpr_req);

void launch_bn_apply(const void* x, const void* res, void* y,
                     const float* stats, const float* gamma,
                     const float* beta, float* rmean, float* rvar,
                     float* smean, float* sinvstd, long M, int C,
                     float momentum, float eps, int training, int act,
                     hipStream_t st);
void launch_bn_apply_f32(const float* ws, const void* res, void* y,
                         void* convout, const float* stats,
                         const float* gamma, const float* beta, float* rmean,
                         float* rvar, float* smean, float* sinvstd, long M,
                         int C, float momentum, float eps, int training,
                         int act, int nsplit, hipStream_t st);
void launch_stats_reduce(const float* ws, float* stats, long M, int C,
                         int nsplit, hipStream_t st);
void launch_stats_bf16_det(const void* x, float* stats, long M, int C,
                           hipStream_t st);
void launch_cast_f32_bf16(const float* src, void* dst, long n, int nsplit,
                          int accum, hipStream_t st);
void launch_cast_bnact(const float* src, void* dst, long M, int C, int nsplit,
                       int accum, const void* x_up, const void* y_up,
                       const float* smean, const float* sinvstd,
                       const float* gamma, const float* beta, float* sum_dz,
                       float* sum_dzx, int mask_mode, hipStream_t st);
void launch_bnact_bwd_reduce(const void* dy, const void* yout, const void* x,
                             const float* smean, const float* sinvstd,
                             const float* gamma, const float* beta,
                             float* sum_dz, float* sum_dzx, long M, int C,
                             int mask_mode, hipStream_t st);
void launch_bn_bwd_apply(const void* dy, const void* yout, const void* x,
                         const float* smean, const float* sinvstd,
                         const float* gamma, const float* beta,
                         const float* sum_dz, const float* sum_dzx,
                         void* dconv, void* dres, long M, int C,
                         int mask_mode, hipStream_t st);
void launch_bn_fwd_owner(const float* ws, const void* res, void* y,
                         void* convout, const float* gamma,
                         const float* beta, float* rmean, float* rvar,
                         float* smean, float* sinvstd, long M, int C,
                         float momentum, float eps, int act, int nsplit,
                         int lpr, hipStream_t st);
void launch_bn_bwd_owner(const void* dy, const void* yout, const void* x,
                         const float* smean, const float* sinvstd,
                         const float* gamma, const float* beta,
                         float* sum_dz, float* sum_dzx, void* dconv,
                         void* dres, long M, int C, int mask_mode, int lpr,
                         hipStream_t st);

void launch_dw_fwd(const void* x, const void* w, void* y, float* stats,
                   int Nb, int H, int W, int C, int Ho, int Wo, int R, int S,
                   int str, int pad, hipStream_t st);
void launch_dw_dgrad(const void* dz, const void* w, void* dx, int Nb, int H,
                     int W, int C, int Ho, int Wo, int R, int S, int str,
                     int pad, hipStream_t st);
void launch_dw_wgrad(const void* x, const void* dz, float* dw, int Nb, int H,
                     int W, int C, int Ho, int Wo, int R, int S, int str,
                     int pad, hipStream_t st);
void launch_maxpool_fwd(const void* x, void* y, unsigned char* idx, int Nb,
                        int H, int W, int C, int Hp, int Wp, hipStream_t st);
void launch_maxpool_bwd(const void* dy, const unsigned char* idx, void* dx,
                        int Nb, int H, int W, int C, int Hp, int Wp,
                        hipStream_t st);
void launch_avgpool_fwd(const void* x, void* y, int Nb, int HW, int C,
                        hipStream_t st);
void launch_avgpool_bwd(const void* dy, void* dx, int Nb, int HW, int C,
                        hipStream_t st);
void launch_linear_fwd(const void* x, const void* w, const float* b, float* y,
                       int B, int In, int Out, hipStream_t st);
void launch_linear_bwd(const float* dy, const void* x, const void* w,
                       void* dx, float* dw, float* db, int B, int In, int Out,
                       int accum, hipStream_t st);
void launch_ce_fwd_bwd(const float* logits, const long* target, float* loss,
                       float* dlogits, int B, int NC, hipStream_t st);
void launch_ce_ls_fwd_bwd(const float* logits, const long* target,
                          float* loss, float* dlogits, int B, int NC,
                          float eps, hipStream_t st);

void launch_adam_step(float* master, float* grad, float* m, float* v,
                      void* shadow, float* step_t, long n, float lr, float b1,
                      float b2, float eps, float wd, int zero_grad,
                      float* extra_zero, long n_extra, const void* gsrc,
                      float gscale, float* prev, float* sumsq, float* divout,
                      hipStream_t st);
void launch_sgd_step(float* master, float* grad, float* mom, void* shadow,
                     long n, float lr, float mu, float wd, int zero_grad,
                     const void* gsrc, float gscale, float* prev,
                     float* sumsq, float* divout, hipStream_t st);
void launch_adam_step_ex(float* master, float* grad, float* m, float* v,
                         void* shadow, float* step_t, long n, float lr,
                         float b1, float b2, float eps, float wd,
                         int zero_grad, float* extra_zero, long n_extra,
                         const void* gsrc, float gscale, float* prev,
                         float* sumsq, float* divout, const float* lr_table,
                         long T, float* lr_out, int decoupled,
                         hipStream_t st);
void launch_sgd_step_ex(float* master, float* grad, float* mom, void* shadow,
                        long n, float lr, float mu, float wd, int zero_grad,
                        const void* gsrc, float gscale, float* prev,
                        float* sumsq, float* divout, float* step_t,
                        const float* lr_table, long T, float* lr_out,
                        int nesterov, hipStream_t st);
void launch_seg_norms(const float* master, const float* grad,
                      const void* gsrc, float gscale, const int* chunks,
                      int nchunks, const int* seg_meta, int nseg,
                      float* partials, float* seg_norms, float* seg_mul,
                      float* norm_out, float wd, float max_norm, int lars,
                      float eta, hipStream_t st);
void launch_adam_step_seg(float* master, float* grad, float* m, float* v,
                          void* shadow, float* step_t, float lr, float b1,
                          float b2, float eps, int zero_grad,
                          float* extra_zero, long n_extra, const void* gsrc,
                          float gscale, float* prev, float* sumsq,
                          float* divout, const float* lr_table, long T,
                          float* lr_out, int decoupled, const int* chunks,
                          int nchunks, const float* seg_mul, hipStream_t st);
void launch_sgd_step_seg(float* master, float* grad, float* mom, void* shadow,
                         float lr, float mu, int zero_grad, const void* gsrc,
                         float gscale, float* prev, float* sumsq,
                         float* divout, float* step_t, const float* lr_table,
                         long T, float* lr_out, int nesterov,
                         const int* chunks, int nchunks, const float* seg_mul,
                         hipStream_t st);

void launch_permute_krsc_rsck(const void* src, void* dst, const int* meta,
                              int nconv, int max_elem, hipStream_t st);
void launch_grad_divergence(const float* g, float* prev, float* sumsq,
                            float* out, long n, int skip_first,
                            hipStream_t st);
void launch_normalize_u8(const void* x, void* y, long total, int C, long HW,
                         float mean, float std, hipStream_t st);
void launch_augment_normalize_u8(const void* x, void* y, void* state,
                                 const int* params, long N, int C, int H,
                                 int W, int pad, int flip, float mean,
                                 float std, hipStream_t st);

}
```

Baseline: 67720 images/sec.

## Clip convolution taps that never overlap the input to shrink reduction depth

```diff
diff --git a/horizonml_amd/ops/csrc/bind.cpp b/horizonml_amd/ops/csrc/bind.cpp
--- a/horizonml_amd/ops/csrc/bind.cpp
+++ b/horizonml_amd/ops/csrc/bind.cpp
@@ -35,6 +35,29 @@
 bool g_wgrad_tr = env_long("HZ_WGRAD_TR", 1) != 0;
 void set_wgrad_tr(bool on) { g_wgrad_tr = on; }
 bool wgrad_tr_enabled() { return g_wgrad_tr; }
+
+bool g_tap_clip = env_long("HZ_TAP_CLIP", 1) != 0;
+void set_tap_clip(bool on) { g_tap_clip = on; }
+bool tap_clip_enabled() { return g_tap_clip; }
+
+std::vector<int64_t> conv_tap_window(int64_t H, int64_t W, int64_t R,
+                                     int64_t S, int64_t stride, int64_t pad) {
+  TORCH_CHECK(stride >= 1 && pad >= 0 && R >= 1 && S >= 1 &&
+                  H + 2 * pad >= R && W + 2 * pad >= S,
+              "conv_tap_window: empty output or bad geometry");
+  ConvP p{};
+  p.H = (int)H;
+  p.W = (int)W;
+  p.C = 1;
+  p.R = p.Rf = (int)R;
+  p.S = p.Sf = (int)S;
+  p.str = (int)stride;
+  p.pad = (int)pad;
+  p.Ho = (p.H + 2 * p.pad - p.R) / p.str + 1;
+  p.Wo = (p.W + 2 * p.pad - p.S) / p.str + 1;
+  p = clip_taps(p);
+  return {p.r0, p.s0, p.R, p.S};
+}
 
 struct PendingWgrad {
   torch::Tensor x, dconv, dw;
@@ -122,6 +145,7 @@
   auto tk3_of = [](const ConvP& p) {
     static const int kd_min = (int)env_long("HZ_WG_TK3_KD", 256);
     static const int m_min = (int)env_long("HZ_WG_TK3_M", 5000);
+    if (taps_clipped(p)) return 64;
     return (p.Kd >= kd_min && p.M >= m_min) ? 128 : 64;
   };
   auto tko_of = [](const ConvP& p) {
@@ -177,6 +201,7 @@
     t.ws = ws_base + ws_off[i];
     t.dW = pend[i].dw.data_ptr<float>();
     t.n = (long)pend[i].p.K * pend[i].p.Kd;
+    wred_set_window(&t, pend[i].p);
     t.msplit = msplit[i];
     t.base = rblocks;
     rblocks += cdiv_i(t.n, 1024);
@@ -222,22 +247,28 @@
                    at::MemoryFormat::ChannelsLast);
 }
 
-ConvP make_convp(const Tensor& x, int K, int R, int S, int stride, int pad) {
+ConvP make_convp(int Nb, int C, int H, int W, int K, int R, int S, int stride,
+                 int pad) {
   ConvP p{};
-  p.Nb = (int)x.size(0);
-  p.C = (int)x.size(1);
-  p.H = (int)x.size(2);
-  p.W = (int)x.size(3);
+  p.Nb = Nb;
+  p.C = C;
+  p.H = H;
+  p.W = W;
   p.K = K;
-  p.R = R;
-  p.S = S;
+  p.R = p.Rf = R;
+  p.S = p.Sf = S;
   p.str = stride;
   p.pad = pad;
   p.Ho = (p.H + 2 * pad - R) / stride + 1;
   p.Wo = (p.W + 2 * pad - S) / stride + 1;
   p.M = p.Nb * p.Ho * p.Wo;
   p.Kd = R * S * p.C;
-  return p;
+  return g_tap_clip ? clip_taps(p) : p;
+}
+
+ConvP make_convp(const Tensor& x, int K, int R, int S, int stride, int pad) {
+  return make_convp((int)x.size(0), (int)x.size(1), (int)x.size(2),
+                    (int)x.size(3), K, R, S, stride, pad);
 }
 
 std::vector<Tensor> conv_bn_act_fwd(
@@ -338,7 +369,7 @@
   TORCH_CHECK(wt.is_contiguous() && wt.scalar_type() == torch::kBFloat16,
               krsc ? "w must be contiguous bf16"
                    : "w_rsck must be contiguous bf16");
-  TORCH_CHECK(wt.numel() == (int64_t)p.K * p.R * p.S * p.C,
+  TORCH_CHECK(wt.numel() == (int64_t)p.K * p.Rf * p.Sf * p.C,
               "dgrad weight has ", wt.numel(), " elements, expected K*R*S*C");
   auto fopt = dconv.options().dtype(torch::kFloat32);
   const int layout = krsc ? DGRAD_W_KRSC : DGRAD_W_RSCK;
@@ -394,20 +425,9 @@
   check_cl(dz, "dz");
   TORCH_CHECK(w.dim() == 4 && w.size(0) == dz.size(1),
               "w must be [K,R,S,C] with K = dz channels");
-  ConvP p{};
-  p.Nb = (int)dz.size(0);
-  p.C = (int)w.size(3);
-  p.H = (int)H;
-  p.W = (int)W;
-  p.K = (int)w.size(0);
-  p.R = (int)w.size(1);
-  p.S = (int)w.size(2);
-  p.str = (int)stride;
-  p.pad = (int)pad;
-  p.Ho = (p.H + 2 * p.pad - p.R) / p.str + 1;
-  p.Wo = (p.W + 2 * p.pad - p.S) / p.str + 1;
-  p.M = p.Nb * p.Ho * p.Wo;
-  p.Kd = p.R * p.S * p.C;
+  const ConvP p = make_convp((int)dz.size(0), (int)w.size(3), (int)H, (int)W,
+                             (int)w.size(0), (int)w.size(1), (int)w.size(2),
+                             (int)stride, (int)pad);
   TORCH_CHECK(dz.size(2) == p.Ho && dz.size(3) == p.Wo,
               "dz spatial size does not match H, W, stride, pad");
   if (dx_accum.has_value()) {
@@ -1293,4 +1313,7 @@
   m.def("dgrad_krsc_enabled", &dgrad_krsc_enabled);
   m.def("set_wgrad_tr", &set_wgrad_tr);
   m.def("wgrad_tr_enabled", &wgrad_tr_enabled);
-}
+  m.def("set_tap_clip", &set_tap_clip);
+  m.def("tap_clip_enabled", &tap_clip_enabled);
+  m.def("conv_tap_window", &conv_tap_window);
+}
diff --git a/horizonml_amd/ops/csrc/conv_kernels.hip b/horizonml_amd/ops/csrc/conv_kernels.hip
--- a/horizonml_amd/ops/csrc/conv_kernels.hip
+++ b/horizonml_amd/ops/csrc/conv_kernels.hip
@@ -1,6 +1,6 @@
 #include "common.h"
 
-template <int MODE>
+template <int MODE, bool CLIP = false>
 DEV int a_addr(const ConvP& p, const MagicP& mg, int m, int k, bool& valid) {
   if (MODE == 0) {
     valid = (m < p.M) & (k < p.Kd);
@@ -10,8 +10,10 @@
     unsigned ho = fdiv(hw, mg, 1), wo = fmod(hw, ho, mg, 1);
     unsigned r = fdiv(k, mg, 2), rm = fmod(k, r, mg, 2);
     unsigned sx = fdiv(rm, mg, 3), c = fmod(rm, sx, mg, 3);
-    int hi = (int)ho * p.str - p.pad + (int)r;
-    int wi = (int)wo * p.str - p.pad + (int)sx;
+    const int ph = CLIP ? p.pad - p.r0 : p.pad;
+    const int pw = CLIP ? p.pad - p.s0 : p.pad;
+    int hi = (int)ho * p.str - ph + (int)r;
+    int wi = (int)wo * p.str - pw + (int)sx;
     valid = (m < p.M) & (k < p.Kd) & (hi >= 0) & (hi < p.H) & (wi >= 0) & (wi < p.W);
     return (((int)n * p.H + hi) * p.W + wi) * p.C + (int)c;
   } else {
@@ -19,7 +21,9 @@
     unsigned hi = fdiv(hw, mg, 1), wi = fmod(hw, hi, mg, 1);
     unsigned r = fdiv(k, mg, 2), rm = fmod(k, r, mg, 2);
     unsigned sx = fdiv(rm, mg, 3), ko = fmod(rm, sx, mg, 3);
-    int hs = (int)hi + p.pad - (int)r, ws = (int)wi + p.pad - (int)sx;
+    const int ph = CLIP ? p.pad - p.r0 : p.pad;
+    const int pw = CLIP ? p.pad - p.s0 : p.pad;
+    int hs = (int)hi + ph - (int)r, ws = (int)wi + pw - (int)sx;
     bool ok = (m < p.M) & (k < p.Kd) & (hs >= 0) & (ws >= 0) &&
               (hs % p.str == 0) && (ws % p.str == 0);
     int ho = hs / p.str, wo = ws / p.str;
@@ -29,25 +33,36 @@
   }
 }
 
-template <int MODE>
+DEV int full_tap(const ConvP& p, const MagicP& mg, int k, int rs) {
+  int r = (int)fdiv(k, mg, 2);
+  return (p.r0 + r) * p.Sf + p.s0 + (rs - r * p.S);
+}
+
+template <int MODE, bool CLIP = false>
 DEV int b_addr(const ConvP& p, const MagicP& mg, int n, int k, int Ntot,
                bool& valid) {
   if (MODE == 2) {
     unsigned rs = fdiv(k, mg, 3), ko = fmod(k, rs, mg, 3);
     valid = (n < Ntot) & (k < p.Kd);
+    if (CLIP) rs = (unsigned)full_tap(p, mg, k, (int)rs);
     return ((int)rs * p.C + n) * p.K + (int)ko;
   }
   valid = (n < Ntot) & (k < p.Kd);
+  if (MODE == 1 && CLIP) {
+    unsigned r = fdiv(k, mg, 2);
+    return n * (p.Rf * p.Sf * p.C) +
+           (p.r0 * p.Sf + p.s0 + (int)r * (p.Sf - p.S)) * p.C + k;
+  }
   return n * p.Kd + k;
 }
 
-template <int MODE, bool VEC>
+template <int MODE, bool VEC, bool CLIP = false>
 DEV V8 load8_a(const bf16* __restrict__ src, const ConvP& p,
                const MagicP& mg, int m, int k) {
   V8 v;
   if (VEC) {
     bool ok;
-    int a = a_addr<MODE>(p, mg, m, k, ok);
+    int a = a_addr<MODE, CLIP>(p, mg, m, k, ok);
     if (ok) v.u = *(const uint4*)(src + a);
     else v.u = uint4{0, 0, 0, 0};
   } else if (MODE == 1) {
@@ -55,7 +70,8 @@
     int ho = hw / p.Wo, wo = hw % p.Wo;
     int r = k / (p.S * p.C), rm = k % (p.S * p.C);
     int s = rm / p.C, c = rm % p.C;
-    int hi = ho * p.str - p.pad + r, wi = wo * p.str - p.pad + s;
+    int hi = ho * p.str - (CLIP ? p.pad - p.r0 : p.pad) + r;
+    int wi = wo * p.str - (CLIP ? p.pad - p.s0 : p.pad) + s;
     const bool mok = m < p.M;
     int kk = k;
 #pragma unroll
@@ -78,26 +94,26 @@
   } else {
     for (int e = 0; e < 8; e++) {
       bool ok;
-      int a = a_addr<MODE>(p, mg, m, k + e, ok);
+      int a = a_addr<MODE, CLIP>(p, mg, m, k + e, ok);
       v.e[e] = ok ? src[a] : (bf16)0.f;
     }
   }
   return v;
 }
 
-template <int MODE, bool VEC>
+template <int MODE, bool VEC, bool CLIP = false>
 DEV V8 load8_b(const bf16* __restrict__ src, const ConvP& p,
                const MagicP& mg, int n, int k, int Ntot) {
   V8 v;
   if (VEC) {
     bool ok;
-    int a = b_addr<MODE>(p, mg, n, k, Ntot, ok);
+    int a = b_addr<MODE, CLIP>(p, mg, n, k, Ntot, ok);
     if (ok) v.u = *(const uint4*)(src + a);
     else v.u = uint4{0, 0, 0, 0};
   } else {
     for (int e = 0; e < 8; e++) {
       bool ok;
-      int a = b_addr<MODE>(p, mg, n, k + e, Ntot, ok);
+      int a = b_addr<MODE, CLIP>(p, mg, n, k + e, Ntot, ok);
       v.e[e] = ok ? src[a] : (bf16)0.f;
     }
   }
@@ -111,13 +127,15 @@
   return k * TN + ((((n >> 4) ^ f)) << 4) + (n & 15);
 }
 
-template <bool VEC>
+template <bool VEC, bool CLIP = false>
 DEV V8 load8_b_krsc(const bf16* __restrict__ src, const ConvP& p,
                     const MagicP& mg, int n, int k, int kend, int Ntot) {
   V8 v;
   unsigned rs = fdiv(k, mg, 3), ko = fmod(k, rs, mg, 3);
   const bool kok = k < kend;
-  const int a = ((int)ko * p.R * p.S + (int)rs) * p.C + n;
+  const int a =
+      CLIP ? ((int)ko * p.Rf * p.Sf + full_tap(p, mg, k, (int)rs)) * p.C + n
+           : ((int)ko * p.R * p.S + (int)rs) * p.C + n;
   if (VEC) {
     if (kok && n < Ntot) v.u = *(const uint4*)(src + a);
     else v.u = uint4{0, 0, 0, 0};
@@ -138,7 +156,7 @@
 #define LDA 40
 
 template <int MODE, bool VECA, bool VECB, bool STATS, bool SPLIT,
-          int TM = 64, int TN = 64, bool KRSC = false>
+          int TM = 64, int TN = 64, bool KRSC = false, bool CLIP = false>
 __global__ __launch_bounds__(256) void k_conv_mfma(
     const bf16* __restrict__ A, const bf16* __restrict__ Bw,
     bf16* __restrict__ Y, float* __restrict__ ws_out,
@@ -168,10 +186,10 @@
 
   auto load_b = [&](int j, int kt) -> V8 {
     if (KRSC)
-      return load8_b_krsc<VECB>(Bw, p, mg, n0 + bncol,
-                                kt + j * BKSTEP + bkrow, kend, Ntot);
-    return load8_b<MODE, VECB>(Bw, p, mg, n0 + j * 64 + srow, kt + scol,
-                               Ntot);
+      return load8_b_krsc<VECB, CLIP>(Bw, p, mg, n0 + bncol,
+                                      kt + j * BKSTEP + bkrow, kend, Ntot);
+    return load8_b<MODE, VECB, CLIP>(Bw, p, mg, n0 + j * 64 + srow,
+                                     kt + scol, Ntot);
   };
   auto store_b = [&](int b, int j, const V8& v) {
     if (KRSC)
@@ -189,7 +207,8 @@
 
 #pragma unroll
   for (int j = 0; j < AC; j++) {
-    V8 a0 = load8_a<MODE, VECA>(A, p, mg, m0 + j * 64 + srow, kbeg + scol);
+    V8 a0 = load8_a<MODE, VECA, CLIP>(A, p, mg, m0 + j * 64 + srow,
+                                      kbeg + scol);
     *(V8*)&As[0][(j * 64 + srow) * LDA + scol] = a0;
   }
 #pragma unroll
@@ -198,8 +217,8 @@
   if (kbeg + 32 < kend) {
 #pragma unroll
     for (int j = 0; j < AC; j++)
-      a_nx[j] = load8_a<MODE, VECA>(A, p, mg, m0 + j * 64 + srow,
-                                    kbeg + 32 + scol);
+      a_nx[j] = load8_a<MODE, VECA, CLIP>(A, p, mg, m0 + j * 64 + srow,
+                                          kbeg + 32 + scol);
 #pragma unroll
     for (int j = 0; j < BC; j++) b_nx[j] = load_b(j, kbeg + 32);
   }
@@ -216,8 +235,8 @@
       if (k0 + 64 < kend) {
 #pragma unroll
         for (int j = 0; j < AC; j++)
-          a_nx[j] = load8_a<MODE, VECA>(A, p, mg, m0 + j * 64 + srow,
-                                        k0 + 64 + scol);
+          a_nx[j] = load8_a<MODE, VECA, CLIP>(A, p, mg, m0 + j * 64 + srow,
+                                              k0 + 64 + scol);
 #pragma unroll
         for (int j = 0; j < BC; j++) b_nx[j] = load_b(j, k0 + 64);
       }
@@ -308,7 +327,7 @@
 };
 using WgradSmem = WgradSmemT<64, 64>;
 
-template <bool VECA, int TK3, int TKO>
+template <bool VECA, int TK3, int TKO, bool CLIP>
 DEV void wgrad_mloop_tr(const bf16* __restrict__ X,
                         const bf16* __restrict__ Dz, const ConvP& p,
                         const MagicP& mg, int Ntot, int k3_0, int n0,
@@ -326,7 +345,8 @@
   auto load_tile = [&](int mt) {
 #pragma unroll
     for (int j = 0; j < AC; j++)
-      a_nx[j] = load8_a<1, VECA>(X, p, mg, mt + sm, k3_0 + j * 64 + sv);
+      a_nx[j] =
+          load8_a<1, VECA, CLIP>(X, p, mg, mt + sm, k3_0 + j * 64 + sv);
 #pragma unroll
     for (int j = 0; j < DC; j++) {
       int m = mt + sm, n = n0 + j * 64 + sv;
@@ -381,7 +401,8 @@
   }
 }
 
-template <bool VECA, int TK3 = 64, int TKO = 64, bool TR = false>
+template <bool VECA, int TK3 = 64, int TKO = 64, bool TR = false,
+          bool CLIP = false>
 DEV void wgrad_tile(const bf16* __restrict__ X, const bf16* __restrict__ Dz,
                     float* __restrict__ out, const ConvP& p,
                     const MagicP& mg, int Ntot, int mchunk, int tx, int ty,
@@ -404,13 +425,14 @@
   f32x4 acc[MI][NI] = {};
 
   if (TR) {
-    wgrad_mloop_tr<VECA, TK3, TKO>(X, Dz, p, mg, Ntot, k3_0, n0, mbeg, mend,
-                                   smem, acc);
+    wgrad_mloop_tr<VECA, TK3, TKO, CLIP>(X, Dz, p, mg, Ntot, k3_0, n0, mbeg,
+                                         mend, smem, acc);
   } else {
   V8 a_nx[AC], d_nx[DC];
 #pragma unroll
   for (int j = 0; j < AC; j++)
-    a_nx[j] = load8_a<1, VECA>(X, p, mg, mbeg + sm, k3_0 + j * 64 + sv);
+    a_nx[j] =
+        load8_a<1, VECA, CLIP>(X, p, mg, mbeg + sm, k3_0 + j * 64 + sv);
 #pragma unroll
   for (int j = 0; j < DC; j++) {
     int m = mbeg + sm, n = n0 + j * 64 + sv;
@@ -441,8 +463,8 @@
     if (m0 + 32 < mend) {
 #pragma unroll
       for (int j = 0; j < AC; j++)
-        a_nx[j] = load8_a<1, VECA>(X, p, mg, m0 + 32 + sm,
-                                   k3_0 + j * 64 + sv);
+        a_nx[j] = load8_a<1, VECA, CLIP>(X, p, mg, m0 + 32 + sm,
+                                         k3_0 + j * 64 + sv);
 #pragma unroll
       for (int j = 0; j < DC; j++) {
         int m = m0 + 32 + sm, n = n0 + j * 64 + sv;
@@ -492,7 +514,30 @@
     }
     __syncthreads();
     const int gko = n0 + pass * 64 + ko_r;
-    if (gko < Ntot) {
+    if (CLIP && !split) {
+      if (gko < Ntot) {
+        const long row = (long)gko * (p.Rf * p.Sf * p.C) +
+                         (p.r0 * p.Sf + p.s0) * p.C;
+        const int skip = (p.Sf - p.S) * p.C;
+        if ((p.C & 3) == 0 && k3_0 + cch + CCH <= p.Kd) {
+#pragma unroll
+          for (int e = 0; e < CCH; e += 4) {
+            const int k3 = k3_0 + cch + e;
+            float* d4 = &dst[row + k3 + (int)fdiv(k3, mg, 2) * skip];
+            float4 v = *(const float4*)&smem.out[ko_r][cch + e];
+            float4 d = *(const float4*)d4;
+            v.x += d.x; v.y += d.y; v.z += d.z; v.w += d.w;
+            *(float4*)d4 = v;
+          }
+        } else {
+          for (int e = 0; e < CCH && k3_0 + cch + e < p.Kd; e++) {
+            const int k3 = k3_0 + cch + e;
+            dst[row + k3 + (int)fdiv(k3, mg, 2) * skip] +=
+                smem.out[ko_r][cch + e];
+          }
+        }
+      }
+    } else if (gko < Ntot) {
       long base = (long)gko * p.Kd + k3_0 + cch;
       if (k3_0 + cch + CCH <= p.Kd) {
 #pragma unroll
@@ -513,18 +558,54 @@
   }
 }
 
-template <bool VECA, bool TR>
+template <bool VECA, bool TR, bool CLIP>
 __global__ __launch_bounds__(256) void k_wgrad(
     const bf16* __restrict__ X, const bf16* __restrict__ Dz,
     float* __restrict__ dW, ConvP p, MagicP mg, int Ntot, int mchunk) {
   __shared__ WgradSmem smem;
-  wgrad_tile<VECA, 64, 64, TR>(X, Dz, dW, p, mg, Ntot, mchunk, blockIdx.x,
-                               blockIdx.y, blockIdx.z, gridDim.z > 1, smem);
-}
-
-__global__ __launch_bounds__(256) void k_wgrad_reduce(
-    const float* __restrict__ ws, float* __restrict__ dW, long n,
-    int msplit) {
+  wgrad_tile<VECA, 64, 64, TR, CLIP>(X, Dz, dW, p, mg, Ntot, mchunk,
+                                     blockIdx.x, blockIdx.y, blockIdx.z,
+                                     gridDim.z > 1, smem);
+}
+
+DEV long wred_dst(const WredTask& t, unsigned i) {
+  unsigned ko = i / (unsigned)t.Kd, k3 = i - ko * (unsigned)t.Kd;
+  return (long)ko * t.KdF + t.org + k3 + (k3 / (unsigned)t.SC) * t.skip;
+}
+
+DEV void wred_scatter(const WredTask& t, long begin, long end, long tid,
+                      long nthr) {
+  if (((t.Kd | t.SC | t.KdF | t.org | t.skip) & 3) == 0) {
+    for (long i4 = begin + tid * 4; i4 < end; i4 += nthr * 4) {
+      float4 v = *(const float4*)&t.ws[i4];
+      for (int z = 1; z < t.msplit; z++) {
+        float4 w = *(const float4*)&t.ws[(long)z * t.n + i4];
+        v.x += w.x; v.y += w.y; v.z += w.z; v.w += w.w;
+      }
+      float4* dp = (float4*)&t.dW[wred_dst(t, (unsigned)i4)];
+      float4 d = *dp;
+      d.x += v.x; d.y += v.y; d.z += v.z; d.w += v.w;
+      *dp = d;
+    }
+  } else {
+    for (long i = begin + tid; i < end; i += nthr) {
+      float v = t.ws[i];
+      for (int z = 1; z < t.msplit; z++) v += t.ws[(long)z * t.n + i];
+      t.dW[wred_dst(t, (unsigned)i)] += v;
+    }
+  }
+}
+
+__global__ __launch_bounds__(256) void k_wgrad_reduce(WredTask t) {
+  if (t.Kd > 0) {
+    wred_scatter(t, 0, t.n, (long)blockIdx.x * blockDim.x + threadIdx.x,
+                 (long)gridDim.x * blockDim.x);
+    return;
+  }
+  const float* __restrict__ ws = t.ws;
+  float* __restrict__ dW = t.dW;
+  const long n = t.n;
+  const int msplit = t.msplit;
   long i4 = ((long)blockIdx.x * blockDim.x + threadIdx.x) * 4;
   long stride = (long)gridDim.x * blockDim.x * 4;
   for (; i4 + 4 <= n; i4 += stride) {
@@ -560,7 +641,17 @@
   __shared__ WgradSmemT<TK3, TKO> smem;
   const bf16* X = (const bf16*)t.X;
   const bf16* Dz = (const bf16*)t.Dz;
-  if (t.vec)
+  constexpr bool CL = TK3 == 64;
+  if (CL && ((t.p.R != t.p.Rf) | (t.p.S != t.p.Sf))) {
+    if (t.vec)
+      wgrad_tile<true, TK3, TKO, TR, CL>(X, Dz, t.out, t.p, t.mg, t.Ntot,
+                                         t.mchunk, tx, ty, z, t.msplit > 1,
+                                         smem);
+    else
+      wgrad_tile<false, TK3, TKO, TR, CL>(X, Dz, t.out, t.p, t.mg, t.Ntot,
+                                          t.mchunk, tx, ty, z, t.msplit > 1,
+                                          smem);
+  } else if (t.vec)
     wgrad_tile<true, TK3, TKO, TR>(X, Dz, t.out, t.p, t.mg, t.Ntot, t.mchunk,
                                    tx, ty, z, t.msplit > 1, smem);
   else
@@ -574,6 +665,11 @@
   int i = 0;
   while (i + 1 < a.n && bid >= a.t[i + 1].base) i++;
   const WredTask& t = a.t[i];
+  if (t.Kd > 0) {
+    const long begin = (long)(bid - t.base) * 1024;
+    wred_scatter(t, begin, min(t.n, begin + 1024), threadIdx.x, 256);
+    return;
+  }
   long i4 = ((long)(bid - t.base) * 256 + threadIdx.x) * 4;
   if (i4 + 4 <= t.n) {
     float4 v = *(const float4*)&t.ws[i4];
@@ -608,6 +704,12 @@
 
 static inline int pick_tile(int M, int N);
 static inline int pick_tile_dgrad(int M, int N);
+static inline int conv_tile(const ConvP& p) {
+  return taps_clipped(p) ? 0 : pick_tile(p.M, p.K);
+}
+static inline int conv_tile_dgrad(const ConvP& p) {
+  return taps_clipped(p) ? 0 : pick_tile_dgrad(p.Nb * p.H * p.W, p.C);
+}
 
 static int sk_fill(int dgrad) {
   static const int vf = (int)env_long("HZ_SK_FILL", 0);
@@ -625,9 +727,18 @@
 
 extern "C" int conv_fwd_splitk(ConvP p) {
   int tiles = cdiv_h(p.K, 64) * cdiv_h(p.M, 64);
+  static const int clip_full = (int)env_long("HZ_SK_CLIP_FULL", 1);
+  if (clip_full && taps_clipped(p)) {
+    const int kd_full = p.Rf * p.Sf * p.C;
+    int sk = pick_splitk(tiles, kd_full);
+    if (sk > 1) {
+      sk = cdiv_h(kd_full, cdiv_h(cdiv_h(kd_full, sk), 32) * 32);
+      sk = min(sk, cdiv_h(p.Kd, 32));
+    }
+    return sk;
+  }
   int sk = pick_splitk(tiles, p.Kd);
-  if (sk == 1 && sk_fill(0) > 0 && p.Kd >= 512
-      && pick_tile(p.M, p.K) == 2) {
+  if (sk == 1 && sk_fill(0) > 0 && p.Kd >= 512 && conv_tile(p) == 2) {
     int blocks = cdiv_h(p.M, 128) * cdiv_h(p.K, 128);
     if (blocks < sk_fill(0)) return fill_splitk(blocks, p.Kd, sk_fill(0));
   }
@@ -641,7 +752,7 @@
   int Kd = p.R * p.S * p.K;
   if (tiles >= tile_min_dg || Kd < kd_min_dg) {
     int M = p.Nb * p.H * p.W;
-    if (sk_fill(1) > 0 && Kd >= 512 && pick_tile_dgrad(M, p.C) == 2) {
+    if (sk_fill(1) > 0 && Kd >= 512 && conv_tile_dgrad(p) == 2) {
       int blocks = cdiv_h(M, 128) * cdiv_h(p.C, 128);
       if (blocks < sk_fill(1)) return fill_splitk(blocks, Kd, sk_fill(1));
     }
@@ -770,8 +881,8 @@
 
 static inline bool stem_eligible(const ConvP& p) {
   static const int on = (int)env_long("HZ_STEM_DIRECT", 0);
-  return on && p.C == 3 && p.R == 7 && p.S == 7 && p.str == 2 &&
-         p.pad == 3 && p.K <= 64 && p.Wo <= 128;
+  return on && !taps_clipped(p) && p.C == 3 && p.R == 7 && p.S == 7 &&
+         p.str == 2 && p.pad == 3 && p.K <= 64 && p.Wo <= 128;
 }
 
 static void launch_stem_conv(const bf16* x, const bf16* w, bf16* y,
@@ -833,22 +944,23 @@
   auto B = (const bf16*)w;
   auto Y = (bf16*)y;
   MagicP mg = make_magic(p, 1);
-  int tile = pick_tile(p.M, p.K);
-#define CASE_T(VA, VB, ST, TM, TN)                                     \
-  k_conv_mfma<1, VA, VB, ST, false, TM, TN><<<grid, 256, 0, st>>>(     \
-      A, B, Y, nullptr, stats, p, mg, p.K, 0, 0)
-#define DISPATCH(TM, TN)                                               \
-  do {                                                                 \
-    dim3 grid(cdiv_h(p.K, TN), cdiv_h(p.M, TM));                       \
-    if (vec && s) CASE_T(true, true, true, TM, TN);                    \
-    else if (vec) CASE_T(true, true, false, TM, TN);                   \
-    else if (s) CASE_T(false, false, true, TM, TN);                    \
-    else CASE_T(false, false, false, TM, TN);                          \
+  int tile = conv_tile(p);
+#define CASE_T(VA, VB, ST, TM, TN, CL)                                    \
+  k_conv_mfma<1, VA, VB, ST, false, TM, TN, false, CL>                    \
+      <<<grid, 256, 0, st>>>(A, B, Y, nullptr, stats, p, mg, p.K, 0, 0)
+#define DISPATCH(TM, TN, CL)                                              \
+  do {                                                                    \
+    dim3 grid(cdiv_h(p.K, TN), cdiv_h(p.M, TM));                          \
+    if (vec && s) CASE_T(true, true, true, TM, TN, CL);                   \
+    else if (vec) CASE_T(true, true, false, TM, TN, CL);                  \
+    else if (s) CASE_T(false, false, true, TM, TN, CL);                   \
+    else CASE_T(false, false, false, TM, TN, CL);                         \
   } while (0)
-  if (tile == 3) DISPATCH(256, 64);
-  else if (tile == 2) DISPATCH(128, 128);
-  else if (tile == 1) DISPATCH(128, 64);
-  else DISPATCH(64, 64);
+  if (tile == 3) DISPATCH(256, 64, false);
+  else if (tile == 2) DISPATCH(128, 128, false);
+  else if (tile == 1) DISPATCH(128, 64, false);
+  else if (taps_clipped(p)) DISPATCH(64, 64, true);
+  else DISPATCH(64, 64, false);
 #undef DISPATCH
 #undef CASE_T
 }
@@ -862,18 +974,27 @@
   auto A = (const bf16*)x;
   auto B = (const bf16*)w;
   MagicP mg = make_magic(p, 1);
-  int tile = pick_tile(p.M, p.K);
-#define SK_T(VA, VB, TM, TN)                                              k_conv_mfma<1, VA, VB, false, true, TM, TN><<<grid, 256, 0, st>>>(          A, B, nullptr, ws, nullptr, p, mg, p.K, kchunk, 0)
-#define DISPATCH(TM, TN)                                                  do {                                                                      dim3 grid(cdiv_h(p.K, TN), cdiv_h(p.M, TM), splitk);                    if (vec) SK_T(true, true, TM, TN);                                      else SK_T(false, false, TM, TN);                                      } while (0)
-  if (tile == 3) DISPATCH(256, 64);
-  else if (tile == 2) DISPATCH(128, 128);
-  else if (tile == 1) DISPATCH(128, 64);
-  else DISPATCH(64, 64);
+  int tile = conv_tile(p);
+#define SK_T(VA, VB, TM, TN, CL)                                        \
+  k_conv_mfma<1, VA, VB, false, true, TM, TN, false, CL>                \
+      <<<grid, 256, 0, st>>>(A, B, nullptr, ws, nullptr, p, mg, p.K,    \
+                             kchunk, 0)
+#define DISPATCH(TM, TN, CL)                                            \
+  do {                                                                  \
+    dim3 grid(cdiv_h(p.K, TN), cdiv_h(p.M, TM), splitk);                \
+    if (vec) SK_T(true, true, TM, TN, CL);                              \
+    else SK_T(false, false, TM, TN, CL);                                \
+  } while (0)
+  if (tile == 3) DISPATCH(256, 64, false);
+  else if (tile == 2) DISPATCH(128, 128, false);
+  else if (tile == 1) DISPATCH(128, 64, false);
+  else if (taps_clipped(p)) DISPATCH(64, 64, true);
+  else DISPATCH(64, 64, false);
 #undef DISPATCH
 #undef SK_T
 }
 
-template <int TM, int TN>
+template <int TM, int TN, bool CL = false>
 static void dgrad_krsc_t(const bf16* A, const bf16* B, bf16* dx, float* ws,
                          bool split, int splitk, int kchunk, const ConvP& p,
                          const MagicP& mg, int accum, hipStream_t st) {
@@ -882,11 +1003,11 @@
 #define KRSC_T(VA, VB)                                                      \
   do {                                                                      \
     if (split)                                                              \
-      k_conv_mfma<2, VA, VB, false, true, TM, TN, true>                     \
+      k_conv_mfma<2, VA, VB, false, true, TM, TN, true, CL>                 \
           <<<grid, 256, 0, st>>>(A, B, nullptr, ws, nullptr, p, mg, p.C,    \
                                  kchunk, 0);                                \
     else                                                                    \
-      k_conv_mfma<2, VA, VB, false, false, TM, TN, true>                    \
+      k_conv_mfma<2, VA, VB, false, false, TM, TN, true, CL>                \
           <<<grid, 256, 0, st>>>(A, B, dx, nullptr, nullptr, p, mg, p.C, 0, \
                                  accum);                                    \
   } while (0)
@@ -911,14 +1032,15 @@
       splitk = cdiv_h(p.Kd, kchunk);
     }
     MagicP mg = make_magic(p, 2);
-    int tile = pick_tile_dgrad(p.M, p.C);
-#define DISPATCH(TM, TN)                                                  \
-  dgrad_krsc_t<TM, TN>(A, B, (bf16*)dx, ws, split, splitk, kchunk, p, mg, \
-                       accum, st)
-    if (tile == 3) DISPATCH(256, 64);
-    else if (tile == 2) DISPATCH(128, 128);
-    else if (tile == 1) DISPATCH(128, 64);
-    else DISPATCH(64, 64);
+    int tile = conv_tile_dgrad(p);
+#define DISPATCH(TM, TN, CL)                                             \
+  dgrad_krsc_t<TM, TN, CL>(A, B, (bf16*)dx, ws, split, splitk, kchunk, p, \
+                           mg, accum, st)
+    if (tile == 3) DISPATCH(256, 64, false);
+    else if (tile == 2) DISPATCH(128, 128, false);
+    else if (tile == 1) DISPATCH(128, 64, false);
+    else if (taps_clipped(p)) DISPATCH(64, 64, true);
+    else DISPATCH(64, 64, false);
 #undef DISPATCH
     return;
   }
@@ -926,31 +1048,42 @@
     int kchunk = cdiv_h(cdiv_h(p.Kd, splitk), 32) * 32;
     splitk = cdiv_h(p.Kd, kchunk);
     MagicP mg = make_magic(p, 2);
-    int tile = pick_tile_dgrad(p.M, p.C);
-#define SKD_T(VA, VB, TM, TN)                                             k_conv_mfma<2, VA, VB, false, true, TM, TN><<<grid, 256, 0, st>>>(          A, B, nullptr, ws, nullptr, p, mg, p.C, kchunk, 0)
-#define DISPATCH(TM, TN)                                                  do {                                                                      dim3 grid(cdiv_h(p.C, TN), cdiv_h(p.M, TM), splitk);                    if (vec) SKD_T(true, true, TM, TN);                                     else SKD_T(false, false, TM, TN);                                     } while (0)
-    if (tile == 3) DISPATCH(256, 64);
-    else if (tile == 2) DISPATCH(128, 128);
-    else if (tile == 1) DISPATCH(128, 64);
-    else DISPATCH(64, 64);
+    int tile = conv_tile_dgrad(p);
+#define SKD_T(VA, VB, TM, TN, CL)                                       \
+  k_conv_mfma<2, VA, VB, false, true, TM, TN, false, CL>                \
+      <<<grid, 256, 0, st>>>(A, B, nullptr, ws, nullptr, p, mg, p.C,    \
+                             kchunk, 0)
+#define DISPATCH(TM, TN, CL)                                            \
+  do {                                                                  \
+    dim3 grid(cdiv_h(p.C, TN), cdiv_h(p.M, TM), splitk);                \
+    if (vec) SKD_T(true, true, TM, TN, CL);                             \
+    else SKD_T(false, false, TM, TN, CL);                               \
+  } while (0)
+    if (tile == 3) DISPATCH(256, 64, false);
+    else if (tile == 2) DISPATCH(128, 128, false);
+    else if (tile == 1) DISPATCH(128, 64, false);
+    else if (taps_clipped(p)) DISPATCH(64, 64, true);
+    else DISPATCH(64, 64, false);
 #undef DISPATCH
 #undef SKD_T
   } else {
     MagicP mg = make_magic(p, 2);
-    int tile = pick_tile_dgrad(p.M, p.C);
-#define DGRAD_T(VA, VB, TM, TN)                                         \
-  k_conv_mfma<2, VA, VB, false, false, TM, TN><<<grid, 256, 0, st>>>(   \
-      A, B, (bf16*)dx, nullptr, nullptr, p, mg, p.C, 0, accum)
-#define DISPATCH(TM, TN)                                                \
+    int tile = conv_tile_dgrad(p);
+#define DGRAD_T(VA, VB, TM, TN, CL)                                     \
+  k_conv_mfma<2, VA, VB, false, false, TM, TN, false, CL>               \
+      <<<grid, 256, 0, st>>>(A, B, (bf16*)dx, nullptr, nullptr, p, mg,  \
+                             p.C, 0, accum)
+#define DISPATCH(TM, TN, CL)                                            \
   do {                                                                  \
     dim3 grid(cdiv_h(p.C, TN), cdiv_h(p.M, TM));                        \
-    if (vec) DGRAD_T(true, true, TM, TN);                               \
-    else DGRAD_T(false, false, TM, TN);                                 \
+    if (vec) DGRAD_T(true, true, TM, TN, CL);                           \
+    else DGRAD_T(false, false, TM, TN, CL);                             \
   } while (0)
-    if (tile == 3) DISPATCH(256, 64);
-    else if (tile == 2) DISPATCH(128, 128);
-    else if (tile == 1) DISPATCH(128, 64);
-    else DISPATCH(64, 64);
+    if (tile == 3) DISPATCH(256, 64, false);
+    else if (tile == 2) DISPATCH(128, 128, false);
+    else if (tile == 1) DISPATCH(128, 64, false);
+    else if (taps_clipped(p)) DISPATCH(64, 64, true);
+    else DISPATCH(64, 64, false);
 #undef DISPATCH
 #undef DGRAD_T
   }
@@ -1015,21 +1148,29 @@
   bool vec = (p.C % 8) == 0;
   float* out = msplit > 1 ? ws : dw;
   MagicP mg = make_magic(p, 1);
-#define WGRAD_T(VA, TR)                                               \
-  k_wgrad<VA, TR><<<grid, 256, 0, st>>>((const bf16*)x, (const bf16*)dz, \
-                                        out, p, mg, p.K, mchunk)
-#define DISPATCH(TR)            \
-  do {                          \
-    if (vec) WGRAD_T(true, TR); \
-    else WGRAD_T(false, TR);    \
+#define WGRAD_T(VA, TR, CL)                                           \
+  k_wgrad<VA, TR, CL><<<grid, 256, 0, st>>>(                          \
+      (const bf16*)x, (const bf16*)dz, out, p, mg, p.K, mchunk)
+#define DISPATCH(TR, CL)            \
+  do {                              \
+    if (vec) WGRAD_T(true, TR, CL); \
+    else WGRAD_T(false, TR, CL);    \
   } while (0)
-  if (tr) DISPATCH(true);
-  else DISPATCH(false);
+  if (taps_clipped(p)) {
+    if (tr) DISPATCH(true, true);
+    else DISPATCH(false, true);
+  } else if (tr) DISPATCH(true, false);
+  else DISPATCH(false, false);
 #undef DISPATCH
 #undef WGRAD_T
   if (msplit > 1) {
-    long n = (long)p.K * p.Kd;
-    int blocks = (int)min((n / 4 + 255) / 256, (long)1024);
-    k_wgrad_reduce<<<blocks, 256, 0, st>>>(ws, dw, n, msplit);
-  }
-}
+    WredTask t{};
+    t.ws = ws;
+    t.dW = dw;
+    t.n = (long)p.K * p.Kd;
+    t.msplit = msplit;
+    wred_set_window(&t, p);
+    int blocks = (int)max(1L, min((t.n / 4 + 255) / 256, (long)1024));
+    k_wgrad_reduce<<<blocks, 256, 0, st>>>(t);
+  }
+}
diff --git a/horizonml_amd/ops/csrc/launch.h b/horizonml_amd/ops/csrc/launch.h
--- a/horizonml_amd/ops/csrc/launch.h
+++ b/horizonml_amd/ops/csrc/launch.h
@@ -9,6 +9,7 @@
   int Ho, Wo, R, S;
   int str, pad;
   int M, Kd;
+  int r0, s0, Rf, Sf;
 };
 
 struct MagicP {
@@ -41,7 +42,17 @@
   long n;
   int msplit;
   int base;
-};
+  int Kd, SC, KdF, org, skip;
+};
+
+inline void wred_set_window(WredTask* t, const ConvP& p) {
+  const bool clipped = p.R != p.Rf || p.S != p.Sf;
+  t->Kd = clipped ? p.Kd : 0;
+  t->SC = p.S * p.C;
+  t->KdF = p.Rf * p.Sf * p.C;
+  t->org = (p.r0 * p.Sf + p.s0) * p.C;
+  t->skip = (p.Sf - p.S) * p.C;
+}
 
 struct WredBatchArgs {
   int n;
@@ -83,6 +94,39 @@
     magic_u32(mg.d[i], &mg.m[i], &mg.s[i]);
   }
   return mg;
+}
+
+inline void tap_range(int H, int Ho, int R, int str, int pad, int* lo,
+                      int* n) {
+  int first = R, last = -1;
+  for (int r = 0; r < R; r++)
+    for (int ho = 0; ho < Ho; ho++) {
+      const int hi = ho * str - pad + r;
+      if (hi >= 0 && hi < H) {
+        if (r < first) first = r;
+        last = r;
+        break;
+      }
+    }
+  *lo = last < 0 ? 0 : first;
+  *n = last < 0 ? 0 : last - first + 1;
+}
+
+inline ConvP clip_taps(ConvP p) {
+  int r0, rn, s0, sn;
+  tap_range(p.H, p.Ho, p.Rf, p.str, p.pad, &r0, &rn);
+  tap_range(p.W, p.Wo, p.Sf, p.str, p.pad, &s0, &sn);
+  if (rn <= 0 || sn <= 0) return p;
+  p.r0 = r0;
+  p.s0 = s0;
+  p.R = rn;
+  p.S = sn;
+  p.Kd = rn * sn * p.C;
+  return p;
+}
+
+inline bool taps_clipped(const ConvP& p) {
+  return p.R != p.Rf || p.S != p.Sf;
 }
 
 inline long env_long(const char* name, long dflt) {
```

New measurement: 71230 images/sec, median of 6. 5.2% higher.
